# zhoubin-me/supertonic

Measured on AMD Instinct MI355X. Metric: audio-sec/sec (RTF^-1), 66M model, batch=128 per GPU, higher is better.
Workload: dtype bf16

## Files before the change

include/stn.h:

```cpp
#ifndef STN_H
#define STN_H
#include <stddef.h>
#include <stdint.h>

#include "stn_arch.h"

#ifdef __cplusplus
extern "C" {
#endif

#define STN_OK 0
#define STN_ERR_INVALID (-1)
#define STN_ERR_DEVICE (-2)
#define STN_ERR_STATE (-3)
#define STN_ERR_UNSUPPORTED (-4)
#define STN_ERR_IO (-5)

#define STN_DTYPE_F32 0
#define STN_DTYPE_BF16 1
#define STN_DTYPE_F16 2

typedef struct stn_handle stn_handle;

typedef struct stn_config {
// ... 233 lines not shown
int stn_expander_curve(const stn_expander* c, int n, const double* in_db, double* out_db);
const char* stn_expander_error(const stn_expander* c, int rate_hz);

int stn_profile_enable(stn_handle* h, int on);
int stn_profile_reset(stn_handle* h);
int stn_profile_filter(stn_handle* h, const char* family_or_null);
int stn_profile_sample(stn_handle* h, int every);
int stn_launch_log_enable(stn_handle* h, int on);
int64_t stn_launch_log(stn_handle* h, char* out, size_t cap);
int stn_profile_count(stn_handle* h);
int stn_profile_get(stn_handle* h, int idx, char* name, size_t name_cap, double* total_ms, int64_t* launches,
                    double* flops, double* bytes);

int stn_dbg_xattn_hs_enable(stn_handle* h, int on);
int64_t stn_dbg_xattn_hs_stamps(stn_handle* h, unsigned long long* out, size_t cap);
int stn_dbg_fold_run_frames(const int32_t* latent_lengths, int B, int n_cu);

int stn_op_gemm(stn_handle* h, int dtype, int M, int N, int K, const float* A , const float* W ,
                const float* bias_or_null, int act , float* out );
int stn_op_gemm_ex(stn_handle* h, int dtype, int M, int N, int K, const float* A , const float* W , int mode, int act,
                   int out_dtype, int ldo, const float* bias_or_null, const float* gamma_or_null, const int32_t* len_or_null, int L,
                   const int32_t* row_b_or_null, const float* rowvec_or_null, int nseq, int nt, int tr, float* out, int64_t out_elems,
                   char* form, size_t form_cap);
int stn_dbg_gemm_form(int dtype, int M, int N, int K, int mode, int out_dtype, int ldo, int masked, int tr, char* out, size_t cap);
int stn_dbg_ffn_form(int dtype, int stage, int C, int I, int64_t M, int64_t gate_rows, int packed, int k, int max_dil, int mask,
                     int64_t min_rows, int64_t split_min_rows, int nt_hints, char* out, size_t cap);
int stn_op_gemm_bench(stn_handle* h, int dtype, int M, int N, int K, int mode, int iters, double* avg_ms);
int stn_op_gemm_phases(stn_handle* h, int dtype, int M, int N, int K, int mode, double* out6);
int stn_op_dwconv_ln(stn_handle* h, int dtype, int B, int L, int C, int k, int dil, const float* x,
                     const float* w , const float* bias, const float* ln_g, const float* ln_b, float* y);
int stn_op_dwconv_ln_ragged(stn_handle* h, int dtype, int B, int L, int C, int k, int dil, const float* x,
                            const float* w , const float* bias, const float* ln_g, const float* ln_b,
                            const int32_t* seqlen , float* y);
int stn_op_dwconv_ln_ex(stn_handle* h, int dtype, int B, int L, int C, int k, int dil, const float* x, int64_t x_rows,
                        const float* w_or_null , const float* bias_or_null, const float* ln_g, const float* ln_b,
                        const int32_t* seqlen_or_null, int packed, int ln_only, float* y, int64_t y_rows, char* form, size_t form_cap);
int stn_op_dwconv_ln_tail(stn_handle* h, int dtype, int B, int L, int C, int k, int dil, const float* x, int64_t x_rows,
                          const float* w , const float* bias, const float* ln_g, const float* ln_b, const int32_t* seqlen,
                          const float* tail , int T, int rf, float* y, int64_t y_rows, char* form, size_t form_cap);
int stn_dbg_dwconv_ln_form(int dtype, int B, int L, int C, int k, int packed, char* out, size_t cap);
int stn_op_fold_ln(stn_handle* h, int dtype, int M, int C, int S, const float* part, const float* b2, const float* gamma,
                   const float* rowvec_or_null, const int32_t* row_b_or_null, int nseq, const float* ln_g, const float* ln_b, float* x,
                   float* y);
int stn_op_layout(stn_handle* h, int which, int dtype, const int32_t* p, int n_p, const float* a, int64_t a_n, const float* b, int64_t b_n,
                  const float* c, int64_t c_n, const int64_t* ids, int64_t ids_n, const int32_t* len, int packed, float* out, int64_t out_n,
                  float* out2, int64_t out2_n, int32_t* iout, int64_t iout_n);
int stn_op_attention(stn_handle* h, int dtype, int B, int Lq, int Lk, int H, int dh, const float* q, const float* k,
                     const float* v, const int32_t* qlen_or_null, const int32_t* klen_or_null, int rope_mode, float* o);
int stn_op_attention_ex(stn_handle* h, int dtype, int B, int Lq, int Lk, int H, int dh, const float* q, int64_t q_elems, int ldq,
                        int q_col, float* kv, int64_t kv_elems, int ldk, int k_col, int v_col, float* o, int64_t o_elems, int ldo,
                        const int32_t* qlen_or_null, const int32_t* klen_or_null, const int32_t* q_off_or_null,
                        const int32_t* k_off_or_null, int rope_mode, int k_rotated, int rot_groups, int rot_stride, int rot_col,
                        char* form, size_t form_cap);
int stn_op_xattn_hs(stn_handle* h, int dtype, int M, const float* xn, const float* Wq, const float* bq_or_null, const float* Wo,
                    const float* kv, int64_t kv_elems, int ldk, int k_col, int B, int L, int Lk, const int32_t* qlen,
                    const int32_t* klen_or_null, const int32_t* k_off_or_null, int rope_mode, int pairs_mode, int64_t part_stride,
                    float* part, int64_t part_elems, int32_t* pairs_out_or_null, char* form, size_t form_cap);
int stn_dbg_attn_form(int kind, int dtype, int B, int Lq, int Lk, int H, int dh, int ldq, int ldk, int misaligned, char* out, size_t cap);
int stn_op_ffn(stn_handle* h, int M, int C, int I, const float* xn , const float* W1, const float* b1, const float* W2,
               const float* b2_or_null, const float* gamma_or_null, const float* rowvec_or_null ,
               const int32_t* row_b_or_null , int nseq, float* x, int fused);
int stn_op_ffn_ex(stn_handle* h, int dtype, int M, int C, int I, const float* xn, int ldx, int64_t xn_elems, const float* W1, const float* b1,
                  const float* W2, const float* b2_or_null, const float* gamma_or_null, const int32_t* len_or_null, int L,
                  const int32_t* row_b_or_null, const float* rowvec_or_null, int rv_ld, int nseq, int mode, int split, float* x, int ldo,
                  int64_t x_elems, float* part_or_null, int64_t part_stride, int64_t part_elems, char* form, size_t form_cap);
int stn_op_ffn_bench(stn_handle* h, int M, int C, int I, int fused, int iters, double* out5);
int stn_op_fold_dwconv_ln(stn_handle* h, int B, int C, int k, int dil, int S, const int32_t* seqlen, const float* x, const float* part,
                          const float* b2_or_null, const float* gamma_or_null, const float* rowvec_or_null , const float* w ,
                          const float* bias, const float* ln_g, const float* ln_b, float* x_out, float* y);
int stn_op_fold_dwconv_ln_ex(stn_handle* h, int dtype, int B, int L, int C, int k, int dil, int S, int run_frames, const int32_t* seqlen,
                             const float* x_in, int64_t x_rows, const float* part, int64_t part_stride, int64_t part_elems,
                             const float* b2_or_null, const float* gamma_or_null, const float* rowvec_or_null, int rv_ld,
// ... 18 lines not shown
```

supertonic_amd/binding.py:

```python
import ctypes
import os

import numpy as np

from .arch import StnArch

_HERE = os.path.dirname(os.path.abspath(__file__))
LIB_PATH = os.environ.get("STN_LIB") or os.path.join(_HERE, "libstn.so")
_LIB = None

F32, BF16, F16 = 0, 1, 2
_DTYPES = {"f32": F32, "fp32": F32, "float32": F32, "bf16": BF16, "f16": F16, "fp16": F16, "float16": F16, "half": F16,
           F32: F32, BF16: BF16, F16: F16}
ACT_NONE, ACT_GELU, ACT_SILU, ACT_GELU_TANH = 0, 1, 2, 3
EPI_STORE, EPI_RESID, EPI_STORE_T = 0, 1, 2
FFN_VOCODER, FFN_ESTIMATOR, FFN_TEXT = 1, 2, 4
LAYOUT_ROW_MAP, LAYOUT_NCL_TO_ROWS, LAYOUT_EULER_NCL, LAYOUT_UNPACK_ROWS, LAYOUT_EMBED, LAYOUT_MASKED_MEAN, LAYOUT_IM2COL, LAYOUT_VOCODER_IN = range(8)
ENC_F32, ENC_PCM16, ENC_PCM24, ENC_MULAW, ENC_ALAW = 0, 1, 2, 3, 4
ENCODINGS = {"f32": ENC_F32, "pcm16": ENC_PCM16, "pcm24": ENC_PCM24, "mulaw": ENC_MULAW, "alaw": ENC_ALAW}
ENCODING_NAMES = {v: k for k, v in ENCODINGS.items()}
ENCODING_BYTES = {ENC_F32: 4, ENC_PCM16: 2, ENC_PCM24: 3, ENC_MULAW: 1, ENC_ALAW: 1}
ZERO_CODEWORD = {ENC_F32: 0, ENC_PCM16: 0, ENC_PCM24: 0, ENC_MULAW: 0xFF, ENC_ALAW: 0xD5}


def encoding_id(enc):
    if isinstance(enc, str) and enc.lower() in ENCODINGS:
        return ENCODINGS[enc.lower()]
    if not isinstance(enc, str) and int(enc) in ENCODING_NAMES:
        return int(enc)
    raise ValueError(f"unknown sample encoding {enc!r}: one of {', '.join(ENCODINGS)}")


def encoded_empty(enc, rows, W):
    e = encoding_id(enc)
    if e == ENC_PCM24:
        return np.empty((rows, W, 3), np.uint8)
    return np.empty((rows, W), {ENC_F32: np.float32, ENC_PCM16: np.int16}.get(e, np.uint8))


JOIN_WHOLE, JOIN_TRIM = 0, 1
JOIN_MODES = {"whole": JOIN_WHOLE, "trim": JOIN_TRIM, JOIN_WHOLE: JOIN_WHOLE, JOIN_TRIM: JOIN_TRIM}
JOIN_GAIN_ROW, JOIN_GAIN_PROG = 0, 1
JOIN_SCOPES = {"row": JOIN_GAIN_ROW, "programme": JOIN_GAIN_PROG, "prog": JOIN_GAIN_PROG, JOIN_GAIN_ROW: JOIN_GAIN_ROW, JOIN_GAIN_PROG: JOIN_GAIN_PROG}


class StnJoin(ctypes.Structure):
    _fields_ = [("n_prog", ctypes.c_int32), ("rows", ctypes.c_void_p), ("gap_samples", ctypes.c_void_p), ("gap_seconds", ctypes.c_void_p),
                ("mode", ctypes.c_int32), ("gain_scope", ctypes.c_int32)]


# ... 489 lines not shown
    L.stn_batch_copy_wav_device.argtypes = [vp, vp, ctypes.c_int64]
    L.stn_batch_copy_pcm16_device.argtypes = [vp, vp, ctypes.c_int64]
    L.stn_profile_filter.argtypes = [vp, ctypes.c_char_p]
    L.stn_profile_sample.argtypes = [vp, ci]
    L.stn_launch_log_enable.argtypes = [vp, ci]
    L.stn_dbg_xattn_hs_enable.argtypes = [vp, ci]
    L.stn_dbg_xattn_hs_stamps.argtypes = [vp, vp, ctypes.c_size_t]
    L.stn_dbg_xattn_hs_stamps.restype = ctypes.c_int64
    L.stn_dbg_fold_run_frames.argtypes = [vp, ctypes.c_int, ctypes.c_int]
    L.stn_dbg_fold_run_frames.restype = ctypes.c_int
    L.stn_dbg_gemm_form.argtypes = [ci, ci, ci, ci, ci, ci, ci, ci, ci, ctypes.c_char_p, ctypes.c_size_t]
    L.stn_dbg_gemm_form.restype = ctypes.c_int
    L.stn_dbg_attn_form.argtypes = [ci, ci, ci, ci, ci, ci, ci, ci, ci, ci, ctypes.c_char_p, ctypes.c_size_t]
    L.stn_dbg_attn_form.restype = ctypes.c_int
    L.stn_dbg_ffn_form.argtypes = [ci, ci, ci, ci, ctypes.c_int64, ctypes.c_int64, ci, ci, ci, ci, ctypes.c_int64, ctypes.c_int64, ci,
                                   ctypes.c_char_p, ctypes.c_size_t]
    L.stn_dbg_ffn_form.restype = ctypes.c_int
    L.stn_launch_log.argtypes = [vp, ctypes.c_char_p, ctypes.c_size_t]
    L.stn_launch_log.restype = ctypes.c_int64
    L.stn_profile_enable.argtypes = [vp, ci]
    L.stn_profile_reset.argtypes = [vp]
    L.stn_profile_count.argtypes = [vp]
    L.stn_profile_get.argtypes = [vp, ci, ctypes.c_char_p, ctypes.c_size_t, ctypes.POINTER(ctypes.c_double),
                                  ctypes.POINTER(ctypes.c_int64), ctypes.POINTER(ctypes.c_double),
                                  ctypes.POINTER(ctypes.c_double)]
    L.stn_op_gemm.argtypes = [vp, ci, ci, ci, ci, _f32p, _f32p, vp, ci, _f32p]
    L.stn_op_gemm_ex.argtypes = [vp, ci, ci, ci, ci, _f32p, _f32p, ci, ci, ci, ci, vp, vp, vp, ci, vp, vp, ci, ci, ci, _f32p,
                                 ctypes.c_int64, ctypes.c_char_p, ctypes.c_size_t]
    L.stn_op_gemm_bench.argtypes = [vp, ci, ci, ci, ci, ci, ci, ctypes.POINTER(ctypes.c_double)]
    L.stn_op_gemm_phases.argtypes = [vp, ci, ci, ci, ci, ci, ctypes.POINTER(ctypes.c_double)]
    L.stn_op_dwconv_ln.argtypes = [vp, ci, ci, ci, ci, ci, ci, _f32p, _f32p, _f32p, _f32p, _f32p, _f32p]
    L.stn_op_dwconv_ln_ragged.argtypes = [vp, ci, ci, ci, ci, ci, ci, _f32p, _f32p, _f32p, _f32p, _f32p, _i32p, _f32p]
    L.stn_op_attention.argtypes = [vp, ci, ci, ci, ci, ci, ci, _f32p, _f32p, _f32p, vp, vp, ci, _f32p]
    L.stn_op_dwconv_ln_ex.argtypes = [vp, ci, ci, ci, ci, ci, ci, _f32p, ctypes.c_int64, vp, vp, _f32p, _f32p, vp, ci, ci, _f32p, ctypes.c_int64,
                                      ctypes.c_char_p, ctypes.c_size_t]
    L.stn_op_dwconv_ln_tail.argtypes = [vp, ci, ci, ci, ci, ci, ci, _f32p, ctypes.c_int64, _f32p, _f32p, _f32p, _f32p, _i32p, _f32p, ci, ci, _f32p,
                                        ctypes.c_int64, ctypes.c_char_p, ctypes.c_size_t]
    L.stn_dbg_resample_form.argtypes = [ci, ci, ctypes.c_int64, ctypes.c_char_p, ctypes.c_size_t]
    L.stn_dbg_resample_form.restype = ctypes.c_int
    L.stn_dbg_dwconv_ln_form.argtypes = [ci, ci, ci, ci, ci, ci, ctypes.c_char_p, ctypes.c_size_t]
    L.stn_dbg_dwconv_ln_form.restype = ctypes.c_int
    L.stn_op_fold_ln.argtypes = [vp, ci, ci, ci, ci, _f32p, _f32p, _f32p, vp, vp, ci, _f32p, _f32p, _f32p, _f32p]
    L.stn_op_layout.argtypes = [vp, ci, ci, _i32p, ci, vp, ctypes.c_int64, vp, ctypes.c_int64, vp, ctypes.c_int64, vp, ctypes.c_int64, vp, ci,
                                vp, ctypes.c_int64, vp, ctypes.c_int64, vp, ctypes.c_int64]
    L.stn_op_attention_ex.argtypes = [vp, ci, ci, ci, ci, ci, ci, _f32p, ctypes.c_int64, ci, ci, _f32p, ctypes.c_int64, ci, ci, ci,
                                      _f32p, ctypes.c_int64, ci, vp, vp, vp, vp, ci, ci, ci, ci, ci, ctypes.c_char_p, ctypes.c_size_t]
    L.stn_op_xattn_hs.argtypes = [vp, ci, ci, _f32p, _f32p, vp, _f32p, _f32p, ctypes.c_int64, ci, ci, ci, ci, ci, _i32p, vp, vp, ci, ci,
                                  ctypes.c_int64, _f32p, ctypes.c_int64, vp, ctypes.c_char_p, ctypes.c_size_t]
    L.stn_op_randn.argtypes = [vp, cu64, ci, ci, ci, vp, vp, _f32p]
    L.stn_op_ffn.argtypes = [vp, ci, ci, ci, _f32p, _f32p, _f32p, _f32p, vp, vp, vp, vp, ci, _f32p, ci]
    L.stn_op_ffn_ex.argtypes = [vp, ci, ci, ci, ci, _f32p, ci, ctypes.c_int64, _f32p, _f32p, _f32p, vp, vp, vp, ci, vp, vp, ci, ci, ci, ci, _f32p, ci,
                                ctypes.c_int64, vp, ctypes.c_int64, ctypes.c_int64, ctypes.c_char_p, ctypes.c_size_t]
    L.stn_op_ffn_bench.argtypes = [vp, ci, ci, ci, ci, ci, ctypes.POINTER(ctypes.c_double)]
    L.stn_set_fused_ffn.argtypes = [vp, ci]
    L.stn_set_fused_ffn_min_rows.argtypes = [vp, ctypes.c_int64, ctypes.c_int64]
    L.stn_op_fold_dwconv_ln.argtypes = [vp, ci, ci, ci, ci, ci, _i32p, _f32p, _f32p, vp, vp, vp, _f32p, _f32p, _f32p, _f32p, _f32p, _f32p]
    L.stn_op_fold_dwconv_ln_ex.argtypes = [vp, ci, ci, ci, ci, ci, ci, ci, ci, _i32p, _f32p, ctypes.c_int64, _f32p, ctypes.c_int64, ctypes.c_int64, vp, vp,
                                           vp, ci, _f32p, _f32p, _f32p, _f32p, _f32p, ctypes.c_int64, _f32p, ctypes.c_int64, ctypes.c_char_p,
                                           ctypes.c_size_t]
    L.stn_dbg_fold_dwconv_ln_form.argtypes = [ci, ci, ci, ci, ci, ci, ci, ci, ci, ctypes.c_char_p, ctypes.c_size_t]
    L.stn_dbg_fold_dwconv_ln_form.restype = ctypes.c_int
    L.stn_op_block_bench.argtypes = [vp, ci, ci, ci, ci, ci, ci, ci, ci, ctypes.POINTER(ctypes.c_double)]
    L.stn_group_create.argtypes = [ci, vp, ci, ctypes.POINTER(vp)]
    L.stn_group_destroy.argtypes = [vp]
    L.stn_group_last_error.restype = ctypes.c_char_p
    L.stn_group_last_error.argtypes = [vp]
    L.stn_group_size.argtypes = [vp]
    L.stn_group_uses_rccl.argtypes = [vp]
    L.stn_group_handle.restype = vp
    L.stn_group_handle.argtypes = [vp, ci]
    L.stn_group_load_synthetic.argtypes = [vp, ctypes.POINTER(StnArch), cu64]
    L.stn_group_load_dir.argtypes = [vp, ctypes.c_char_p]
    L.stn_group_deal.argtypes = [ci, _i32p, ci, _i32p, _i32p]
    L.stn_group_synthesize.argtypes = [vp, ci, ci, _i64p, _f32p, _f32p, _f32p, ci, cf, vp, cu64, ctypes.POINTER(ctypes.c_int64)]
# ... 527 lines not shown
    r = load().stn_dbg_fold_run_frames(a.ctypes.data, len(a), int(n_cu))
    if r < 0:
        raise StnError(r, "stn_dbg_fold_run_frames: bad arguments")
    return int(r)


def gemm_form(dtype, M, N, K, mode=EPI_STORE, out_dtype="f32", ldo=None, masked=False, tr=-1):
    buf = ctypes.create_string_buffer(128)
    r = load().stn_dbg_gemm_form(_DTYPES[dtype], int(M), int(N), int(K), int(mode), _DTYPES[out_dtype], int(N if ldo is None else ldo),
                                 int(bool(masked)), int(tr), buf, len(buf))
    if r < 0:
        raise StnError(r, "stn_dbg_gemm_form: the launcher refuses this call")
    return buf.value.decode()


def attn_form(dtype, B, Lq, Lk, H, dh, ldq=None, ldk=None, misaligned=0, kind=0):
    buf = ctypes.create_string_buffer(64)
    C = H * dh
    r = load().stn_dbg_attn_form(int(kind), _DTYPES[dtype], int(B), int(Lq), int(Lk), int(H), int(dh), int(C if ldq is None else ldq),
                                 int(C if ldk is None else ldk), int(misaligned), buf, len(buf))
    if r < 0:
        raise StnError(r, "stn_dbg_attn_form: the launcher refuses this call")
    return buf.value.decode()


def dwconv_ln_form(dtype, B, L, C, k, packed=False):
    buf = ctypes.create_string_buffer(32)
    r = load().stn_dbg_dwconv_ln_form(_DTYPES[dtype], int(B), int(L), int(C), int(k), int(bool(packed)), buf, len(buf))
    if r < 0:
        raise StnError(r, "stn_dbg_dwconv_ln_form: the launcher refuses this call")
    return buf.value.decode()


def fold_dwconv_ln_form(dtype, B, L, C, k, dil, S, rowvec=True, run_frames=0):
    buf = ctypes.create_string_buffer(96)
    r = load().stn_dbg_fold_dwconv_ln_form(_DTYPES[dtype], int(B), int(L), int(C), int(k), int(dil), int(S), int(bool(rowvec)), int(run_frames),
                                           buf, len(buf))
    if r < 0:
        raise StnError(r, "stn_dbg_fold_dwconv_ln_form: the launcher refuses this call")
    return buf.value.decode()


def ffn_form(dtype, stage, C, I, M, gate_rows=0, packed=True, k=5, max_dil=1, mask=9, min_rows=18432, split_min_rows=1, nt_hints=True):
    buf = ctypes.create_string_buffer(32)
    r = load().stn_dbg_ffn_form(_DTYPES[dtype], int(stage), int(C), int(I), int(M), int(gate_rows), int(bool(packed)), int(k), int(max_dil),
                                int(mask), int(min_rows), int(split_min_rows), int(bool(nt_hints)), buf, len(buf))
    if r < 0:
        raise StnError(r, "stn_dbg_ffn_form: invalid arguments")
    return buf.value.decode()


def _c(a, dt):
    return np.ascontiguousarray(a, dtype=dt)


def _opt(a, dt):
    if a is None:
        return None, None
    arr = _c(a, dt)
    return arr, arr.ctypes.data


class Engine:

    def __init__(self, device=0, dtype="bf16"):
        self._lib = load()
# ... 903 lines not shown
        self._ck(self._lib.stn_op_fold_dwconv_ln_ex(self._h, self.dtype if dtype is None else _DTYPES[dtype], len(seqlen), int(L), C, w.shape[1], int(dil),
                                                    int(S), int(run_frames), seqlen, x_in.reshape(-1), x_in.shape[0], part, int(part_stride), part.size,
                                                    b2p, gp, vp_, C if _v is None else _v.shape[1], w, _c(bias, np.float32), _c(g, np.float32),
                                                    _c(b, np.float32), xo.reshape(-1), xo.shape[0], yo.reshape(-1), yo.shape[0], form, ctypes.sizeof(form)))
        return xo, yo, form.value.decode()

    def op_block_bench(self, B, L, C, I, k, dil, mode, iters=20):
        out = (ctypes.c_double * 6)()
        self._ck(self._lib.stn_op_block_bench(self._h, B, L, C, I, k, dil, mode, iters, out))
        return dict(ms=out[0], conv_ms=out[1], fold_phase1=out[2], fold_barrier=out[3], fold_phase2=out[4], fold_span=out[5])

    def set_fused_ffn_min_rows(self, k4_rows=-1, split_rows=-1):
        self._ck(self._lib.stn_set_fused_ffn_min_rows(self._h, int(k4_rows), int(split_rows)))

    def op_gemm_phases(self, M, N, K, mode=0, dtype=None):
        out = (ctypes.c_double * 6)()
        self._ck(self._lib.stn_op_gemm_phases(self._h, self.dtype if dtype is None else _DTYPES[dtype], M, N, K, mode, out))
        return dict(first_stage=out[0], k_loop=out[1], epilogue=out[2], grid_span=out[3], entry_spread=out[4], workgroups=int(out[5]))

    def op_dwconv_ln(self, x, w, bias, g, b, dil, dtype=None, seqlen=None):
        B, L, C = x.shape
        k = w.shape[1]
        y = np.empty((B, L, C), np.float32)
        if seqlen is not None:
            self._ck(self._lib.stn_op_dwconv_ln_ragged(self._h, self.dtype if dtype is None else _DTYPES[dtype], B, L, C, k,
                                                       dil, _c(x, np.float32), _c(w, np.float32), _c(bias, np.float32),
                                                       _c(g, np.float32), _c(b, np.float32), _c(seqlen, np.int32), y))
            return y
        self._ck(self._lib.stn_op_dwconv_ln(self._h, self.dtype if dtype is None else _DTYPES[dtype], B, L, C, k, dil,
                                            _c(x, np.float32), _c(w, np.float32), _c(bias, np.float32),
                                            _c(g, np.float32), _c(b, np.float32), y))
        return y

    def op_dwconv_ln_ex(self, x, w, bias, g, b, dil, out, B, L, seqlen=None, packed=False, ln_only=False, dtype=None):
        x = _c(x, np.float32)
        o_r = np.array(out, dtype=np.float32, order="C", copy=True)
        C = x.shape[1]
        _w, wp = _opt(w, np.float32)
        _b, bp = _opt(bias, np.float32)
        _l, lp = _opt(seqlen, np.int32)
        form = ctypes.create_string_buffer(32)
        self._ck(self._lib.stn_op_dwconv_ln_ex(self._h, self.dtype if dtype is None else _DTYPES[dtype], int(B), int(L), C,
                                               1 if _w is None else _w.shape[1], int(dil), x.reshape(-1), x.shape[0], wp, bp, _c(g, np.float32),
                                               _c(b, np.float32), lp, int(bool(packed)), int(bool(ln_only)), o_r.reshape(-1), o_r.shape[0], form,
                                               ctypes.sizeof(form)))
        return o_r, form.value.decode()

    def op_dwconv_ln_tail(self, x, w, bias, g, b, dil, out, L, seqlen, tail, T, dtype=None):
        x = _c(x, np.float32)
        tail = _c(tail, np.float32)
        o_r = np.array(out, dtype=np.float32, order="C", copy=True)
        C = x.shape[1]
        w = _c(w, np.float32)
        seqlen = _c(seqlen, np.int32)
        assert tail.ndim == 2 and tail.shape[1] == C and tail.shape[0] >= 1
        form = ctypes.create_string_buffer(32)
        self._ck(self._lib.stn_op_dwconv_ln_tail(self._h, self.dtype if dtype is None else _DTYPES[dtype], len(seqlen), int(L), C, w.shape[1],
                                                 int(dil), x.reshape(-1), x.shape[0], w, _c(bias, np.float32), _c(g, np.float32),
                                                 _c(b, np.float32), seqlen, tail.reshape(-1), int(T), tail.shape[0] - 1, o_r.reshape(-1),
                                                 o_r.shape[0], form, ctypes.sizeof(form)))
        return o_r, form.value.decode()

    def op_fold_ln(self, x, part, b2, gamma, g, b, rowvec=None, row_b=None, dtype=None):
        x_r = np.array(x, dtype=np.float32, order="C", copy=True)
        M, C = x_r.shape
        part = _c(part, np.float32)
# ... 91 lines not shown
```

supertonic_amd/csrc/api.cpp:

```cpp
#include "../../include/stn.h"

#include <algorithm>
#include <complex>
#include <cstdio>
#include <cstring>
#include <fstream>
#include <string>

#include "engine.hpp"
#include "host/json_min.hpp"
#include "host/graph_bind.hpp"
#include "host/onnx_reader.hpp"

#include <map>
#include <sstream>

struct stn_handle {
    stn::Engine* eng = nullptr;
    std::string err;
    std::vector<std::pair<std::string, stn::KernelStat>> prof;
};

static thread_local std::string g_create_err;

// ... 879 lines not shown
}
int stn_dbg_ffn_form(int dtype, int stage, int C, int I, int64_t M, int64_t gate_rows, int packed, int k, int max_dil, int mask,
                     int64_t min_rows, int64_t split_min_rows, int nt_hints, char* out, size_t cap) {
    if (C < 1 || I < 1 || M < 1 || k < 1 || max_dil < 1 || (stage != stn::FFN_VOCODER && stage != stn::FFN_ESTIMATOR && stage != stn::FFN_TEXT) ||
        (dtype != STN_DTYPE_F32 && dtype != STN_DTYPE_BF16 && dtype != STN_DTYPE_F16))
        return STN_ERR_INVALID;
    const std::string f = stn::ffn_form(dtype, stage, C, I, M, gate_rows, packed != 0, k, max_dil, mask, min_rows, split_min_rows, nt_hints != 0).str();
    if (out && cap > f.size()) std::memcpy(out, f.c_str(), f.size() + 1);
    return (int)f.size();
}
int stn_op_gemm_bench(stn_handle* h, int dtype, int M, int N, int K, int mode, int iters, double* avg_ms) {
    STN_TRY(h, { need(M > 0 && N > 0 && K > 0 && iters > 0 && avg_ms, "stn_op_gemm_bench: bad argument");
                 need(K % (dtype != STN_DTYPE_F32 ? 8 : 4) == 0, "K must be a multiple of 8 (bf16) / 4 (f32)");
                 *avg_ms = h->eng->op_gemm_bench(dtype, M, N, K, mode, iters); })
}
int stn_op_gemm_phases(stn_handle* h, int dtype, int M, int N, int K, int mode, double* out6) {
    STN_TRY(h, { need(M > 0 && N > 0 && K > 0 && out6, "stn_op_gemm_phases: bad argument");
                 need(K % (dtype != STN_DTYPE_F32 ? 8 : 4) == 0, "K must be a multiple of 8 (bf16) / 4 (f32)");
                 h->eng->op_gemm_phases(dtype, M, N, K, mode, out6); })
}
int stn_op_dwconv_ln(stn_handle* h, int dtype, int B, int L, int C, int k, int dil, const float* x, const float* w,
                     const float* bias, const float* g, const float* b, float* y) {
    STN_TRY(h, { need(B > 0 && L > 0 && C > 0 && C % 4 == 0 && C <= 1024 && k > 0 && (k & 1) && dil > 0 && x && w && bias && g && b && y,
                      "stn_op_dwconv_ln: bad argument");
                 h->eng->op_dwconv_ln(dtype, B, L, C, k, dil, x, w, bias, g, b, y); })
}
int stn_op_dwconv_ln_ragged(stn_handle* h, int dtype, int B, int L, int C, int k, int dil, const float* x, const float* w,
                            const float* bias, const float* g, const float* b, const int32_t* seqlen, float* y) {
    STN_TRY(h, { need(B > 0 && L > 0 && C > 0 && C % 4 == 0 && C <= 1024 && k > 0 && (k & 1) && dil > 0 && x && w && bias && g && b && y && seqlen,
                      "stn_op_dwconv_ln_ragged: bad argument");
                 for (int i = 0; i < B; ++i) need(seqlen[i] >= 0 && seqlen[i] <= L, "stn_op_dwconv_ln_ragged: seqlen out of [0, L]");
                 h->eng->op_dwconv_ln(dtype, B, L, C, k, dil, x, w, bias, g, b, y, seqlen); })
}
static void dwconv_ln_ex_checked(stn_handle* h, int dtype, int B, int L, int C, int k, int dil, const float* x, int64_t x_rows, const float* w,
                                 const float* bias, const float* g, const float* b, const int32_t* seqlen, int packed, int ln_only, float* y,
                                 int64_t y_rows, char* form, size_t form_cap) {
    need(B > 0 && L > 0 && C > 0 && C % 4 == 0 && C <= 1024 && k > 0 && (k & 1) && dil > 0 && x && g && b && y && x_rows > 0 && y_rows > 0,
         "stn_op_dwconv_ln_ex: bad argument");
    need(dtype == STN_DTYPE_F32 || dtype == STN_DTYPE_BF16 || dtype == STN_DTYPE_F16, "stn_op_dwconv_ln_ex: unknown dtype");
    need(ln_only || (w && bias), "stn_op_dwconv_ln_ex: the conv needs w and bias");
    need(!(packed && ln_only), "stn_op_dwconv_ln_ex: ln_only takes no packed layout");
    need(!packed || (seqlen && B <= 1024), "stn_op_dwconv_ln_ex: packed rows need seqlen and B <= 1024");
    int64_t rows = (int64_t)B * L;
    if (seqlen && !ln_only) {
        int64_t tot = 0;
        for (int i = 0; i < B; ++i) { need(seqlen[i] >= 0 && seqlen[i] <= L, "stn_op_dwconv_ln_ex: seqlen out of [0, L]"); tot += seqlen[i]; }
        if (packed) rows = tot;
    }
    need(x_rows >= rows && y_rows >= rows, "stn_op_dwconv_ln_ex: x / y hold fewer rows than the launch addresses");
    const std::string f = h->eng->op_dwconv_ln_ex(dtype, B, L, C, k, dil, x, x_rows, w, bias, g, b, ln_only ? nullptr : seqlen, packed, ln_only, y, y_rows);
    if (form && form_cap) std::snprintf(form, form_cap, "%s", f.c_str());
}
int stn_op_dwconv_ln_ex(stn_handle* h, int dtype, int B, int L, int C, int k, int dil, const float* x, int64_t x_rows, const float* w,
                        const float* bias, const float* g, const float* b, const int32_t* seqlen, int packed, int ln_only, float* y,
                        int64_t y_rows, char* form, size_t form_cap) {
    STN_TRY(h, dwconv_ln_ex_checked(h, dtype, B, L, C, k, dil, x, x_rows, w, bias, g, b, seqlen, packed, ln_only, y, y_rows, form, form_cap))
}
static void dwconv_ln_tail_checked(stn_handle* h, int dtype, int B, int L, int C, int k, int dil, const float* x, int64_t x_rows, const float* w,
                                   const float* bias, const float* g, const float* b, const int32_t* seqlen, const float* tail, int T, int rf,
                                   float* y, int64_t y_rows, char* form, size_t form_cap) {
    need(B > 0 && B <= 1024 && L > 0 && C > 0 && C % 4 == 0 && C <= 512 && (k == 5 || k == 7) && dil > 0 && x && w && bias && g && b && y && seqlen &&
             x_rows > 0 && y_rows > 0,
         "stn_op_dwconv_ln_tail: bad argument");
    need(dtype == STN_DTYPE_F32 || dtype == STN_DTYPE_BF16 || dtype == STN_DTYPE_F16, "stn_op_dwconv_ln_tail: unknown dtype");
    need(tail && rf >= 0 && T >= L, "stn_op_dwconv_ln_tail: needs a tail table of rf + 1 >= 1 rows and T >= L");
    int64_t rows = 0;
    for (int i = 0; i < B; ++i) { need(seqlen[i] >= 0 && seqlen[i] <= L, "stn_op_dwconv_ln_tail: seqlen out of [0, L]"); rows += seqlen[i]; }
    need(x_rows >= rows && y_rows >= rows, "stn_op_dwconv_ln_tail: x / y hold fewer rows than the launch addresses");
    const std::string f = h->eng->op_dwconv_ln_ex(dtype, B, L, C, k, dil, x, x_rows, w, bias, g, b, seqlen, 1, 0, y, y_rows, tail, T, rf);
    if (form && form_cap) std::snprintf(form, form_cap, "%s", f.c_str());
}
int stn_op_dwconv_ln_tail(stn_handle* h, int dtype, int B, int L, int C, int k, int dil, const float* x, int64_t x_rows, const float* w,
                          const float* bias, const float* g, const float* b, const int32_t* seqlen, const float* tail, int T, int rf, float* y,
                          int64_t y_rows, char* form, size_t form_cap) {
    STN_TRY(h, dwconv_ln_tail_checked(h, dtype, B, L, C, k, dil, x, x_rows, w, bias, g, b, seqlen, tail, T, rf, y, y_rows, form, form_cap))
}
int stn_dbg_dwconv_ln_form(int dtype, int B, int L, int C, int k, int packed, char* out, size_t cap) {
    if (B < 1 || L < 1 || C < 1 || k < 1 || !(k & 1) || (dtype != STN_DTYPE_F32 && dtype != STN_DTYPE_BF16 && dtype != STN_DTYPE_F16)) return STN_ERR_INVALID;
    std::string f;
    try { f = stn::dwconv_ln_form(dtype, B, L, C, k, packed != 0).str(); } catch (const std::exception&) { return STN_ERR_INVALID; }
    if (out && cap > f.size()) std::memcpy(out, f.c_str(), f.size() + 1);
    return (int)f.size();
}
int stn_op_fold_ln(stn_handle* h, int dtype, int M, int C, int S, const float* part, const float* b2, const float* gamma, const float* rowvec,
                   const int32_t* row_b, int nseq, const float* g, const float* b, float* x, float* y) {
    STN_TRY(h, { need(M > 0 && C > 0 && C % 4 == 0 && C <= 1024 && (S == 4 || S == 8 || S == 12 || S == 24) && part && b2 && gamma && g && b && x && y,
                      "stn_op_fold_ln: bad argument");
                 need(dtype == STN_DTYPE_BF16 || dtype == STN_DTYPE_F16, "stn_op_fold_ln: a 16-bit format needed");
                 need(!rowvec || nseq > 0, "stn_op_fold_ln: rowvec needs nseq > 0");
                 if (rowvec && row_b) for (int m = 0; m < M; ++m) need(row_b[m] >= 0 && row_b[m] < nseq, "stn_op_fold_ln: row_b out of range");
                 h->eng->op_fold_ln(dtype, M, C, S, part, b2, gamma, rowvec, row_b, nseq, g, b, x, y); })
}
int stn_op_layout(stn_handle* h, int which, int dtype, const int32_t* p, int n_p, const float* a, int64_t a_n, const float* b, int64_t b_n,
                  const float* c, int64_t c_n, const int64_t* ids, int64_t ids_n, const int32_t* len, int packed, float* out, int64_t out_n,
                  float* out2, int64_t out2_n, int32_t* iout, int64_t iout_n) {
    static const int n_params[8] = {3, 4, 5, 3, 4, 3, 6, 6};
    STN_TRY(h, { need(which >= 0 && which < 8 && p && n_p == n_params[which], "stn_op_layout: unknown kernel or parameter count");
                 need(dtype == STN_DTYPE_F32 || dtype == STN_DTYPE_BF16 || dtype == STN_DTYPE_F16, "stn_op_layout: unknown dtype");
                 need(a_n >= 0 && b_n >= 0 && c_n >= 0 && ids_n >= 0 && out_n >= 0 && out2_n >= 0 && iout_n >= 0 && (a || !a_n) && (b || !b_n) && (c || !c_n) &&
                          (ids || !ids_n) && (out || !out_n) && (out2 || !out2_n) && (iout || !iout_n),
                      "stn_op_layout: a buffer without a pointer");
                 h->eng->op_layout(which, dtype, p, a, a_n, b, b_n, c, c_n, ids, ids_n, len, packed, out, out_n, out2, out2_n, iout, iout_n); })
}
int stn_op_attention(stn_handle* h, int dtype, int B, int Lq, int Lk, int H, int dh, const float* q, const float* k,
                     const float* v, const int32_t* qlen, const int32_t* klen, int rope_mode, float* o) {
    STN_TRY(h, { need(B > 0 && Lq > 0 && Lk > 0 && H > 0 && dh >= 8 && dh % 8 == 0 && dh <= 96 && q && k && v && o,
                      "stn_op_attention: bad argument");
                 h->eng->op_attention(dtype, B, Lq, Lk, H, dh, q, k, v, qlen, klen, rope_mode, o); })
}
static void attention_ex_checked(stn_handle* h, int dtype, int B, int Lq, int Lk, int H, int dh, const float* q, int64_t q_elems, int ldq,
                                 int q_col, float* kv, int64_t kv_elems, int ldk, int k_col, int v_col, float* o, int64_t o_elems, int ldo,
                                 const int32_t* qlen, const int32_t* klen, const int32_t* q_off, const int32_t* k_off, int rope_mode,
                                 int k_rotated, int rot_groups, int rot_stride, int rot_col, char* form, size_t form_cap) {
    need(B > 0 && Lq > 0 && Lk > 0 && H > 0 && dh >= 8 && dh % 8 == 0 && dh <= 96 && q && kv && o, "stn_op_attention_ex: bad argument");
    need(dtype == STN_DTYPE_F32 || dtype == STN_DTYPE_BF16 || dtype == STN_DTYPE_F16, "stn_op_attention_ex: unknown dtype");
    need(rope_mode >= -1 && rope_mode <= 1, "stn_op_attention_ex: rope_mode must be -1, 0 or 1");
    const int64_t C = (int64_t)H * dh;
    need(ldq > 0 && ldk > 0 && ldo >= C && q_col >= 0 && k_col >= 0 && v_col >= 0 && q_col + C <= ldq && k_col + C <= ldk && v_col + C <= ldk,
         "stn_op_attention_ex: the heads must lie inside the rows (col + H*dh <= ld, ldo >= H*dh)");
    need((q_off == nullptr || qlen) && (k_off == nullptr || klen), "stn_op_attention_ex: packed rows need their lengths");
    const int64_t qrows = q_elems / ldq, krows = kv_elems / ldk, orows = o_elems / ldo;
    for (int b = 0; b < B; ++b) {
        need(!qlen || qlen[b] >= 0, "stn_op_attention_ex: qlen < 0");
        need(!klen || klen[b] >= 0, "stn_op_attention_ex: klen < 0");
        if (q_off)
            need(qlen[b] <= Lq && q_off[b] >= 0 && (int64_t)q_off[b] + qlen[b] <= std::min(qrows, orows),
                 "stn_op_attention_ex: packed query rows outside q / o (or qlen > Lq)");
        if (k_off) need(k_off[b] >= 0 && (int64_t)k_off[b] + std::min(klen[b], Lk) <= krows, "stn_op_attention_ex: packed key rows outside kv");
    }
    if (!q_off) need((int64_t)B * Lq <= std::min(qrows, orows), "stn_op_attention_ex: q / o hold fewer than B*Lq rows");
// ... 168 lines not shown
```

supertonic_amd/csrc/engine.cpp:

```cpp
#include "engine.hpp"
#include "dev_env.hpp"
#include "engine_internal.hpp"

#include <algorithm>
#include <cmath>
#include <cstdio>
#include <cstring>

namespace stn {
using detail::up;

Arena::~Arena() {
    for (auto& c : chunks_) (void)hipFree(c.p);
}
size_t Arena::capacity() const {
    size_t t = 0;
    for (auto& c : chunks_) t += c.cap;
    return t;
}
void* Arena::alloc(size_t bytes) {
    bytes = (bytes + 255) & ~size_t(255);
    if (bytes == 0) bytes = 256;
    for (;;) {
        if (cur_ < chunks_.size()) {
// ... 105 lines not shown
        if (g.exec2) (void)hipGraphExecDestroy(g.exec2);
        if (g.graph2) (void)hipGraphDestroy(g.graph2);
    }
    graphs_.clear();
    warm_keys_.clear();
}

void Engine::free_weights() {
    if (s_) (void)hipStreamSynchronize(s_);
    drop_graphs();
    ++wgen_;
    for (void* p : owned_) (void)hipFree(p);
    owned_.clear();
    w_.clear();
    frag_w_.clear();
    ffn_w_.clear();
    loaded_ = false;
    params_ = 0;
}

Engine::~Engine() {
    (void)hipSetDevice(device_);
    if (s_) (void)hipStreamSynchronize(s_);
    if (dp_s_) (void)hipStreamSynchronize(dp_s_);
    if (te_s_) (void)hipStreamSynchronize(te_s_);
    free_weights();
    for (void* p : batch_owned_) (void)hipFree(p);
    for (void* p : batch_retired_) (void)hipFree(p);
    free_vocoder_constants();
    if (tcond_.buf) (void)hipFree(tcond_.buf);
    for (auto& sp : spans_) { (void)hipEventDestroy(sp.a); (void)hipEventDestroy(sp.b); }
    for (auto ev : ev_pool_) (void)hipEventDestroy(ev);
    drop_graphs();
    if (pin_llen_) (void)hipHostFree(pin_llen_);
    if (pin_seed_) (void)hipHostFree(pin_seed_);
    if (seed_dev_) (void)hipFree(seed_dev_);
    rs_release();
    fl_release();
    xp_release();
    ds_release();
    cp_release();
    lo_release();
    for (auto& f : fetch_) {
        if (f.busy && f.done) (void)hipEventSynchronize(f.done);
        if (f.dev) (void)hipFree(f.dev);
        if (f.pin) (void)hipHostFree(f.pin);
        if (f.ready) (void)hipEventDestroy(f.ready);
        if (f.done) (void)hipEventDestroy(f.done);
    }
    if (copy_s_) (void)hipStreamDestroy(copy_s_);
    if (own_s_) (void)hipStreamDestroy(own_s_);
    if (dp_s_) (void)hipStreamDestroy(dp_s_);
    if (te_s_) (void)hipStreamDestroy(te_s_);
    if (ev_te_) (void)hipEventDestroy(ev_te_);
    if (ev_copied_) (void)hipEventDestroy(ev_copied_);
    if (ev_dp_) (void)hipEventDestroy(ev_dp_);
}

DevTensor& Engine::tensor(const std::string& name) {
    auto it = w_.find(name);
    if (it == w_.end()) throw std::runtime_error("unknown weight tensor: " + name);
    return it->second;
}
Linear Engine::linear(const std::string& p) {
    Linear l;
    l.w = tensor(p + ".w");
    l.b = tensor(p + ".b").f32;
    l.N = l.w.rows;
    l.K = l.w.cols;
// ... 548 lines not shown
float* Engine::ve_time_cond_dev(int rows, const float* total_step, const float* current_step, float* tb_out) {
    stage_ = "ve";
    const stn_arch& a = a_;
    const int C = a.ve_dim, nb = a.ve_main_blocks;
    float* tb = tb_out ? tb_out : f32_alloc((int64_t)rows * nb * C);
    const Arena::Mark mk = ar_.mark();
    float* te = f32_alloc((int64_t)rows * a.ve_time_dim);
    launch_time_embed(s_, current_step, total_step, rows, a.ve_time_dim, a.time_scale, te);
    float* t1 = f32_alloc((int64_t)rows * C);
    Epilogue et1; et1.mode = EPI_STORE; et1.act = ACT_SILU; et1.out_dtype = F32; et1.out = t1; et1.ldo = C;
    gemm("gemm_small_f32", F32, te, a.ve_time_dim, linear("ve.t1"), rows, et1);
    float* tc = f32_alloc((int64_t)rows * C);
    Epilogue et2; et2.mode = EPI_STORE; et2.out_dtype = F32; et2.out = tc; et2.ldo = C;
    gemm("gemm_small_f32", F32, t1, C, linear("ve.t2"), rows, et2);
    Epilogue et3; et3.mode = EPI_STORE; et3.out_dtype = F32; et3.out = tb; et3.ldo = nb * C;
    gemm("gemm_small_f32", F32, tc, C, linear("ve.time_all"), rows, et3);
    ar_.release(mk);
    return tb;
}

void Engine::ve_step_dev(int B, int L, const VeCtx& c, const float* noisy, const int* tlen, const int* llen,
                         const float* total_step, const float* current_step, float* denoised, const float* tb, const Ragged* rg,
                         const float* dt, void* z_rows, bool z_ready, bool z_next) {
    stage_ = "ve";
    const stn_arch& a = a_;
    const int C = a.ve_dim, D = a.latent_dim * a.chunk_compress_factor, nb = a.ve_main_blocks, H = a.ve_heads;
    const int64_t M = rg ? (int64_t)rg->rows : (int64_t)B * L;
    const int* rmask = rg ? nullptr : llen;
    const int* roff = rg ? rg->off : nullptr;
    const size_t esz = is_half(dt_) ? 2 : 4;
    const Arena::Mark mk = ar_.mark();
    const int Dp = (D + 63) / 64 * 64;
    void* z = z_rows ? z_rows : act_alloc(M * Dp);
    if (!(z_rows && z_ready)) launch_ncl_to_rows(s_, dt_, noisy, B, D, L, z, Dp, llen, roff);
    const FfnForm ff = ffn_plan(FFN_ESTIMATOR, C, a.ve_hidden, M, 0, rg != nullptr, a.ve_kernel, 1 << std::max(0, a.ve_dilated - 1));
    const bool split = ff.kind == FFN_K4_SPLIT;
    FoldState fs;
    fs.x = f32_alloc(M * C);
    if (split) {
        fs.x_alt = f32_alloc(M * C);
        fs.part_stride = ffn_split_rows(M) * C;
        fs.part = act_alloc(fs.part_stride * std::max(ff.split, H));
    }
    FoldState* const fsp = split ? &fs : nullptr;
    Epilogue ein; ein.mode = EPI_STORE; ein.out_dtype = F32; ein.out = fs.x; ein.ldo = C; ein.len = rmask; ein.L = L;
    gemm("gemm_in", dt_, z, Dp, linear("ve.in_pad"), (int)M, ein);
    if (!tb) tb = ve_time_cond_dev(B, total_step, current_step);

    auto cross = [&](const std::string& p, const void* kv_all, int blk, int Lk, const int* klen, int rope_mode) {
        const Attn w = attn_w(p, false);
        const char* kp0 = static_cast<const char*>(kv_all) + (size_t)blk * 2 * C * esz;
        const auto fq = frag_w_.find(w.q.w.as(dt_));
        const auto foa = frag_acc_w_.find(w.o.w.as(dt_));
        if (fused_xattn_ && split && unit_vec_ && C <= 1024 && fq != frag_w_.end() && foa != frag_acc_w_.end() && xattn_hs_supported(dt_, C, H, L, Lk, nb * 2 * C)) {
            const Arena::Mark m2 = ar_.mark();
            void* xn = act_alloc(M * C);
            fold_layernorm(fs, M, C, w.ln, xn, "layernorm");
            if (kv_all == c.text_kv && text_gate_) { auto fire = std::move(text_gate_); text_gate_ = nullptr; fire(); }
            if (prof_on_) prof_begin("xattn_hs", 4.0 * M * (double)C * C + 4.0 * M * (double)Lk * C,
                                     (double)M * C * (esz + 2.0 * H) + 2.0 * C * C * esz + (double)B * Lk * 2 * C * esz);
            unsigned long long* ts = nullptr;
            if (hs_ts_ && (int64_t)(B + 8) * H <= HS_TS_WG) { ts = hs_ts_; hs_ts_wgs_ = (B + 8) * H; }
            launch_xattn_hs(s_, dt_, xn, M, fq->second, w.q.b, kp0, kp0 + (size_t)C * esz, nb * 2 * C, foa->second, fs.part, fs.part_stride, B, L, Lk,
                            llen, klen, roff, kv_all == c.text_kv ? c.text_off : nullptr, rope_mode, a.rope_base, a.larope_gamma, ts, rg->hs_pairs);
            if (prof_on_) prof_end();
            fs.pending = true;
            fs.fold = FoldArgs{};
// ... 18 lines not shown
                         a.larope_gamma, rope_mode >= 0, roff, kv_all == c.text_kv ? c.text_off : nullptr);
        if (prof_on_) prof_end();
        Epilogue eo; eo.mode = EPI_RESID; eo.resid = x; eo.ldo = C; eo.len = rmask; eo.L = L;
        gemm("gemm_attn_out", dt_, o, C, w.o, (int)M, eo);
        ar_.release(m2);
    };

    for (int blk = 0; blk < nb; ++blk) {
        const std::string p = "ve.m" + std::to_string(blk);
        for (int j = 0; j < a.ve_dilated; ++j) {
            const bool last = j == a.ve_dilated - 1;
            convnext(convnext_w(p + ".dil" + std::to_string(j)), ff, fs.x, B, L, C, a.ve_hidden, a.ve_kernel, 1 << j, llen, nullptr,
                     last ? tb + (size_t)blk * C : nullptr, nb * C, rg, fsp);
        }
        if (a.ve_dilated == 0) launch_add_rowvec(s_, fs.x, tb + (size_t)blk * C, nb * C, B, L, C, llen);
        convnext(convnext_w(p + ".cn_a"), ff, fs.x, B, L, C, a.ve_hidden, a.ve_kernel, 1, llen, nullptr, nullptr, 0, rg, fsp);
        cross(p + ".text", c.text_kv, blk, c.Lt, tlen, 1);
        convnext(convnext_w(p + ".cn_b"), ff, fs.x, B, L, C, a.ve_hidden, a.ve_kernel, 1, llen, nullptr, nullptr, 0, rg, fsp);
        cross(p + ".style", c.style_kv, blk, a.n_style_ttl, nullptr, -1);
    }
    for (int j = 0; j < a.ve_tail_blocks; ++j)
        convnext(convnext_w("ve.tail" + std::to_string(j)), ff, fs.x, B, L, C, a.ve_hidden, a.ve_kernel, 1, llen, nullptr, nullptr, 0, rg, fsp);
    void* xn = act_alloc(M * C);
    fold_layernorm(fs, M, C, lnorm("ve.out_ln"), xn, nullptr);
    const float* dtv = dt;
    if (!dtv) {
        float* d = f32_alloc(B);
        launch_reciprocal(s_, total_step, B, d);
        dtv = d;
    }
    float* vel = f32_alloc(M * D);
    Epilogue eo; eo.mode = EPI_STORE; eo.out_dtype = F32; eo.out = vel; eo.ldo = D;
    gemm("gemm_out", dt_, xn, C, linear("ve.out"), (int)M, eo);
    launch_euler_ncl(s_, noisy, vel, dtv, llen, B, D, L, denoised, roff, (z_rows && z_next) ? z_rows : nullptr, dt_, Dp);
    ar_.release(mk);
}

int Engine::vocoder_receptive_field() const {
    int rf = (a_.vo_in_kernel - 1) / 2;
    for (int i = 0; i < a_.vo_blocks; ++i) rf += (a_.vo_kernel - 1) / 2 * a_.vo_dilations[i];
    return rf;
}

void Engine::hs_stamps_enable(bool on) {
    sync();
    drop_graphs();
    if (on && !hs_ts_) {
        void* d = nullptr;
        STN_HIP(hipMalloc(&d, sizeof(unsigned long long) * 8 * HS_TS_WG));
        STN_HIP(hipMemset(d, 0, sizeof(unsigned long long) * 8 * HS_TS_WG));
        hs_ts_ = static_cast<unsigned long long*>(d);
    } else if (!on && hs_ts_) {
        (void)hipFree(hs_ts_);
        hs_ts_ = nullptr;
    }
    hs_ts_wgs_ = 0;
}
int64_t Engine::hs_stamps_fetch(unsigned long long* out, size_t cap) {
    if (!hs_ts_) return 0;
    sync();
    const size_t n = std::min(cap, (size_t)hs_ts_wgs_ * 8);
    if (out && n) STN_HIP(hipMemcpy(out, hs_ts_, n * sizeof(unsigned long long), hipMemcpyDeviceToHost));
    return hs_ts_wgs_;
}

void Engine::prepare_xattn_weights() {
    frag_w_.clear();
// ... 117 lines not shown
}

int Engine::trimmed_rows(int B, int L, std::vector<int>* n_host) const {
    if (!packed_ve_ || vo_ragged_ || !vo_c_[0].quiet || vo_rf_ <= 0 || B > 1024) return 0;
    const int ccf = a_.chunk_compress_factor, T = L * ccf, rf = vo_rf_;
    long tot = 0;
    bool any = false;
    for (int i = 0; i < B; ++i) {
        const int l6 = bt_.h_llen[i] * ccf;
        const bool trim = l6 + 2 * rf <= T;
        any = any || trim;
        const int n = trim ? l6 + 2 * rf : T;
        if (n_host) n_host->push_back(n);
        tot += n;
    }
    return (any && tot * 10 <= (long)B * T * 9) ? (int)tot : 0;
}

int Engine::tail_rows(int B, int L) const {
    if (!packed_ve_ || vo_ragged_ || !vo_c_[0].tail || vo_rf_ <= 0 || B > 1024) return 0;
    const int ccf = a_.chunk_compress_factor, T = L * ccf, rf = vo_rf_;
    long tot = 0;
    for (int i = 0; i < B; ++i) tot += std::min(bt_.h_llen[i] * ccf + rf, T);
    return tot * 10 <= (long)B * T * 9 ? (int)tot : 0;
}

int Engine::vocoder_rows(int B, int L, int* form) const {
    int rows = trimmed_rows(B, L, nullptr);
    *form = rows ? VO_TRIM_2RF : VO_DENSE;
    if (!rows && (rows = tail_rows(B, L))) *form = VO_TRIM_TAIL;
    return rows;
}

void Engine::vocoder_dev(int B, int L, const float* latent, float* wav, const int* vlen, int vrows, const int* valid, bool tails) {
    stage_ = "vo";
    const stn_arch& a = a_;
    const int C = a.vo_dim, T = L * a.chunk_compress_factor;
    const bool packed = vlen && vrows > 0 && is_half(dt_) && B <= 1024 && dwconv_ln_supports_packed(C, a.vo_kernel);
    if (valid && !packed) throw std::runtime_error("trimmed vocoder needs the packed bf16 path");
    if (tails && !valid) throw std::logic_error("vocoder_dev: the tail form is a trimmed form");
    const int64_t M = packed ? (int64_t)vrows : (int64_t)B * T;
    const Arena::Mark mk = ar_.mark();
    Ragged rg;
    if (packed) {
        int* off = static_cast<int*>(ar_.alloc(sizeof(int) * (size_t)(B + 1)));
        launch_row_map(s_, vlen, B, off, nullptr);
        rg.off = off; rg.rows = vrows;
    }
    const Ragged* rgp = packed ? &rg : nullptr;
    float* x = f32_alloc(M * C);
    if (is_half(dt_)) {
        const int kp = (a.latent_dim * a.vo_in_kernel + 63) / 64 * 64;
        void* cols = act_alloc(M * kp);
        launch_vocoder_im2col(s_, dt_, latent, B, L, a.latent_dim, a.chunk_compress_factor, a.vo_in_kernel, kp, cols, vlen,
                              packed ? rg.off : nullptr);
        Linear lin;
        lin.w = tensor("vo.in_gemm.w"); lin.b = vecf("vo.in.b"); lin.N = C; lin.K = kp;
        Epilogue ei; ei.mode = EPI_STORE; ei.out_dtype = F32; ei.out = x; ei.ldo = C;
        gemm("gemm_in", dt_, cols, kp, lin, (int)M, ei);
    } else {
        if (prof_on_) prof_begin("vocoder_in", 2.0 * M * C * a.latent_dim * a.vo_in_kernel, (double)M * (a.latent_dim + C) * 4.0);
        launch_vocoder_in(s_, latent, B, L, a.latent_dim, a.chunk_compress_factor, vecf("vo.in.wt"), vecf("vo.in.b"), C,
                          a.vo_in_kernel, x, vlen);
        if (prof_on_) prof_end();
    }
    FfnForm ff = ffn_plan(FFN_VOCODER, C, a.vo_hidden, M, valid ? (int64_t)B * T : 0, packed, a.vo_kernel,
                          a.vo_blocks ? *std::max_element(a.vo_dilations, a.vo_dilations + a.vo_blocks) : 1);
    if (vo_force_ffn_ >= 0) ff = FfnForm{vo_force_ffn_, 1, false};
    const VoConsts& vc = vo_c_[ff.kind == FFN_K4];
    if (valid && !(vc.quiet && vc.edge && vc.tail)) throw std::logic_error("vocoder_dev: no zero-latent constants for form " + ff.str());
    DwconvTail tl;
    for (int i = 0; i < a.vo_blocks; ++i) {
        if (vo_capture_) {
            const int rf = vocoder_receptive_field();
            for (int j = 0; j <= rf; ++j)
                STN_HIP(hipMemcpyAsync(vo_capture_ + ((size_t)i * (rf + 1) + j) * C, x + (size_t)(M - 1 - j) * C, sizeof(float) * (size_t)C,
                                       hipMemcpyDeviceToDevice, s_));
        }
        if (tails) { tl.tail = vc.tail + (size_t)i * (vo_rf_ + 1) * C; tl.T = T; tl.rf = vo_rf_; }
        convnext(convnext_w("vo.blk" + std::to_string(i)), ff, x, B, T, C, a.vo_hidden, a.vo_kernel, a.vo_dilations[i],
                 packed ? vlen : nullptr, packed ? nullptr : vlen, nullptr, 0, rgp, nullptr, tl);
    }
    void* xn = act_alloc(M * C);
    const LNorm ln = lnorm("vo.out_ln");
    launch_layernorm(s_, dt_, x, M, C, ln.g, ln.b, a.ln_eps, xn);
    if (packed) {
        float* wp = f32_alloc(M * a.base_chunk_size);
        Epilogue e; e.mode = EPI_STORE; e.out_dtype = F32; e.out = wp; e.ldo = a.base_chunk_size;
        gemm("gemm_head", dt_, xn, C, linear("vo.head"), (int)M, e);
        if (prof_on_) prof_begin("unpack_rows", 0.0, ((double)M + (double)B * T) * a.base_chunk_size * 4.0);
        if (valid) launch_unpack_rows_quiet(s_, wp, valid, rg.off, B, T, a.base_chunk_size, vo_rf_, vc.quiet, vc.edge, wav);
        else launch_unpack_rows(s_, wp, vlen, rg.off, B, T, a.base_chunk_size, wav);
        if (prof_on_) prof_end();
    } else {
        Epilogue e; e.mode = EPI_STORE; e.out_dtype = F32; e.out = wav; e.ldo = a.base_chunk_size; e.len = vlen; e.L = T;
        gemm("gemm_head", dt_, xn, C, linear("vo.head"), (int)M, e);
    }
    ar_.release(mk);
}


void Engine::duration(int B, int Lt, const int64_t* ids, const float* style_dp, const float* text_mask, float* dur) {
    STN_HIP(hipSetDevice(device_));
    ar_.reset();
    int64_t* d_ids = up(ar_, s_, ids, (size_t)B * Lt);
    float* d_mask = up(ar_, s_, text_mask, (size_t)B * Lt);
    float* d_st = up(ar_, s_, style_dp, (size_t)B * a_.n_style_dp * a_.d_style_dp);
    int* tlen = static_cast<int*>(ar_.alloc(sizeof(int) * B));
    float* d_dur = f32_alloc(B);
    launch_mask_to_len(s_, d_mask, B, Lt, tlen);
    duration_dev(B, Lt, d_ids, d_st, tlen, d_dur);
    STN_HIP(hipMemcpyAsync(dur, d_dur, sizeof(float) * B, hipMemcpyDeviceToHost, s_));
    sync();
}

void Engine::text_enc(int B, int Lt, const int64_t* ids, const float* style_ttl, const float* text_mask, float* text_emb) {
    STN_HIP(hipSetDevice(device_));
    ar_.reset();
    int64_t* d_ids = up(ar_, s_, ids, (size_t)B * Lt);
    float* d_mask = up(ar_, s_, text_mask, (size_t)B * Lt);
    float* d_st = up(ar_, s_, style_ttl, (size_t)B * a_.n_style_ttl * a_.d_style_ttl);
    int* tlen = static_cast<int*>(ar_.alloc(sizeof(int) * B));
    const size_t n = (size_t)B * a_.te_out_dim * Lt;
    float* d_out = f32_alloc(n);
    launch_mask_to_len(s_, d_mask, B, Lt, tlen);
    text_enc_dev(B, Lt, d_ids, d_st, tlen, d_out, nullptr);
// ... 44 lines not shown
```

supertonic_amd/csrc/engine.hpp:

```cpp
#pragma once
#include <cmath>
#include <hip/hip_runtime.h>

#include <cstdint>
#include <functional>
#include <iterator>
#include <stdexcept>
#include <string>
#include <unordered_map>
#include <vector>

#include "../../include/stn_arch.h"
#include "host/join_plan.hpp"
#include "host/pause_plan.hpp"
#include "host/pitch.hpp"
#include "kernels.hpp"

namespace stn {

#define STN_HIP(expr)                                                                                          \
    do {                                                                                                       \
        hipError_t e_ = (expr);                                                                                \
        if (e_ != hipSuccess)                                                                                  \
            throw std::runtime_error(std::string("HIP error: ") + hipGetErrorString(e_) + " at " #expr);       \
    } while (0)

struct DevTensor {
    float* f32 = nullptr;
    uint16_t* bf16 = nullptr;
    int rows = 0, cols = 0;
    const void* as(int dt) const { return is_half(dt) ? static_cast<const void*>(bf16) : static_cast<const void*>(f32); }
};

struct Linear { DevTensor w; const float* b = nullptr; int N = 0, K = 0; };
struct LNorm { const float* g = nullptr; const float* b = nullptr; };
struct ConvNeXt { const float* dw_t = nullptr; const float* dw_b = nullptr; LNorm ln; Linear pw1, pw2; const float* gamma = nullptr; };
struct Attn { LNorm ln; Linear q, kv, qkv, o; };

class Arena {
   public:
    struct Mark { size_t chunk, off; };
    Arena() = default;
    Arena(const Arena&) = delete;
    Arena& operator=(const Arena&) = delete;
    ~Arena();
// ... 76 lines not shown
    void load_synthetic(const stn_arch& a, uint64_t seed);
    using TensorSource = std::function<std::vector<float>(const std::string& name, int rows, int cols)>;
    void load_tensors(const stn_arch& a, const TensorSource& src);
    std::vector<std::string> tensor_names(const stn_arch& a);
    bool loaded() const { return loaded_; }
    const stn_arch& arch() const { return a_; }
    int64_t param_count() const { return params_; }
    int dtype() const { return dt_; }
    hipStream_t stream() const { return s_; }
    void sync() { STN_HIP(hipStreamSynchronize(s_)); if (dp_s_) STN_HIP(hipStreamSynchronize(dp_s_)); if (te_s_) STN_HIP(hipStreamSynchronize(te_s_)); }
    void set_stream(hipStream_t s);

    struct Ragged;
    void duration_dev(int B, int Lt, const int64_t* ids, const float* style_dp, const int* tlen, float* dur, const Ragged* trg = nullptr);
    void text_enc_dev(int B, int Lt, const int64_t* ids, const float* style_ttl, const int* tlen, float* ncl, void* rows,
                      const Ragged* trg = nullptr);
    struct VeCtx { void* text_kv = nullptr; void* style_kv = nullptr; int Lt = 0; const int* text_off = nullptr; };
    VeCtx ve_prepare_dev(int B, int Lt, const void* text_rows, const float* style_ttl, const int* tlen, const Ragged* trg = nullptr, bool defer_text = false);
    void ve_text_kv_dev(const VeCtx& c, int B, int Lt, const void* text_rows, const int* tlen, const Ragged* trg);
    float* ve_time_cond_dev(int rows, const float* total_step, const float* current_step, float* tb_out = nullptr );
    struct TimeCond { int steps = 0, B = 0; uint64_t wgen = ~0ull; float* buf = nullptr; size_t cap = 0; float *tot = nullptr, *cur = nullptr, *dt = nullptr, *tb = nullptr; };
    TimeCond tcond_;
    void ensure_time_cond(int total_step, int B);
    struct Ragged { const int* off = nullptr; const int* row_b = nullptr; int rows = 0;
                    const int* hs_pairs = nullptr;
                    int fold_run = 0; };
    void ve_step_dev(int B, int L, const VeCtx& c, const float* noisy, const int* tlen, const int* llen,
                     const float* total_step, const float* current_step, float* denoised, const float* tb = nullptr,
                     const Ragged* rg = nullptr, const float* dt = nullptr ,
                     void* z_rows = nullptr ,
                     bool z_ready = false ,
                     bool z_next = false );
    void vocoder_dev(int B, int L, const float* latent, float* wav, const int* vlen = nullptr, int vrows = 0,
                     const int* valid = nullptr, bool tails = false);
    int vocoder_receptive_field() const;
    void prepare_xattn_weights();
    std::unordered_map<const void*, const void*> frag_w_;
    void hs_stamps_enable(bool on);
    int64_t hs_stamps_fetch(unsigned long long* out, size_t cap);
    unsigned long long* hs_ts_ = nullptr;
    int hs_ts_wgs_ = 0;
    static constexpr int HS_TS_WG = 8192;
    const float* unit_vec_ = nullptr;
    std::unordered_map<const void*, const void*> frag_acc_w_;
    void prepare_vocoder_constants();
    void prepare_ffn_weights();
    struct FfnW { const void *wseq = nullptr, *wsplit[std::size(FFN_SPLITS)] = {}; };
    std::unordered_map<const void*, FfnW> ffn_w_;

    void duration(int B, int Lt, const int64_t* ids, const float* style_dp, const float* text_mask, float* dur);
    void text_enc(int B, int Lt, const int64_t* ids, const float* style_ttl, const float* text_mask, float* text_emb);
    void vector_est(int B, int L, int Lt, const float* noisy, const float* text_emb, const float* style_ttl,
                    const float* text_mask, const float* latent_mask, const float* total_step,
                    const float* current_step, float* denoised);
    void vocoder(int B, int L, const float* latent, float* wav);

    struct Batch {
        int B = 0, Lt = 0, L = 0, noise_L = 0, total_step = 0;
        float speed = 1.f;
        bool have_override = false, have_noise = false;
        uint64_t noise_seed = 0;
        int64_t* ids = nullptr; size_t ids_cap = 0;
        int* tlen = nullptr; size_t tlen_cap = 0;
        float* style_ttl = nullptr; size_t ttl_cap = 0;
        float* style_dp = nullptr; size_t dp_cap = 0;
        float* dur = nullptr; size_t dur_cap = 0;
        int* llen = nullptr; size_t llen_cap = 0;
        int64_t* utt_ids = nullptr; size_t utt_cap = 0;
        float* noise = nullptr; size_t noise_cap = 0;
        float* xt[2] = {nullptr, nullptr}; size_t xt_cap[2] = {0, 0};
        float* wav = nullptr; size_t wav_cap = 0;
        unsigned char* text_side = nullptr; size_t text_side_cap = 0;
        unsigned char* text_rows = nullptr; size_t text_cap = 0;
        int* toff = nullptr; size_t toff_cap = 0;
        int trows = 0;
        uint64_t gen = 0;
        std::vector<float> h_dur; std::vector<int> h_llen;
    };
    void batch_upload(int B, int Lt, const int64_t* ids, const float* text_mask, const float* style_ttl,
                      const float* style_dp, const float* duration_override, const int64_t* utt_ids);
    void batch_set_noise(const float* noise, int L);
    void batch_run(int total_step, float speed, uint64_t noise_seed);
    void set_graph_mode(bool on) { graph_on_ = on; }
    void set_vocoder_mode(bool length_aware) { vo_ragged_ = length_aware; }
    void set_packed_rows(bool on) { packed_ve_ = on; }
    void set_gelu_form(int tanh_form) { if ((tanh_form != 0) != (gelu_act_ == ACT_GELU_TANH)) { sync(); drop_graphs(); } gelu_act_ = tanh_form ? ACT_GELU_TANH : ACT_GELU; }
    int gelu_form() const { return gelu_act_ == ACT_GELU_TANH ? 1 : 0; }
    void set_shape_buckets(bool on) { shape_buckets_ = on; }
    static int64_t bucket_up(int64_t x, int64_t min_gran) {
        if (x <= 0) return x;
        int64_t g = min_gran;
        while (g * 8 <= x) g *= 2;
        return (x + g - 1) / g * g;
    }
    void set_duration_read(bool always) { dur_read_always_ = always; }
    void set_fused_xattn(int mode) { fused_xattn_ = mode ? 1 : 0; }
    void set_fused_ffn(int mask) { fused_ffn_ = mask; }
    void set_fused_ffn_min_rows(int64_t k4_rows, int64_t split_rows) {
        sync(); drop_graphs();
        if (k4_rows >= 0) ffn_min_rows_ = k4_rows;
// ... 146 lines not shown
    void set_expander(bool on, const stn_expander* c);
    bool expander_on() const { return xp_on_; }
    const stn_expander& expander() const { return xp_set_; }
    void batch_expander(float* min_attenuation_db, int64_t* closed_samples);
    struct XpProbe {
        int x_misalign = 0, in_place = 0;
        float *open = nullptr, *s1_end = nullptr, *s1_start = nullptr, *s2_end = nullptr, *s2_start = nullptr;
        bool guard_ok = false;
        const char* form = "";
    };
    void op_expander(int hz, int rows, int W, const float* x, const stn_expander& c, float* y, XpProbe* probe);

    void profile_enable(bool on) { if (on != prof_on_) profile_reset(); prof_on_ = on; }
    void launch_log_enable(bool on);
    std::string launch_log() const;
    void profile_sample(int every) { prof_every_ = every < 1 ? 1 : every; prof_seen_ = 0; }
    void profile_filter(const std::string& family) { if (family != prof_filter_) profile_reset(); prof_filter_ = family; }
    void profile_reset();
    std::vector<std::pair<std::string, KernelStat>> profile_collect();

    void op_gemm(int dtype, int M, int N, int K, const float* A, const float* W, const float* bias, int act, float* out);
    std::string op_gemm_ex(int dtype, int M, int N, int K, const float* A, const float* W, int mode, int act, int out_dtype, int ldo,
                           const float* bias, const float* gamma, const int* len, int L, const int* row_b, const float* rowvec, int nseq,
                           int nt, int tr, float* out, int64_t out_elems);
    std::string op_attention_ex(int dtype, int B, int Lq, int Lk, int H, int dh, const float* q, int64_t q_elems, int ldq, int q_col,
                                float* kv, int64_t kv_elems, int ldk, int k_col, int v_col, float* o, int64_t o_elems, int ldo,
                                const int* qlen, const int* klen, const int* q_off, const int* k_off, int rope_mode, int k_rotated,
                                int rot_groups, int rot_stride, int rot_col);
    std::string op_xattn_hs(int dtype, int M, const float* xn, const float* Wq, const float* bq, const float* Wo, const float* kv,
                            int64_t kv_elems, int ldk, int k_col, int B, int L, int Lk, const int* qlen, const int* klen, const int* k_off,
                            int rope_mode, int pairs_mode, int64_t part_stride, float* part, int64_t part_elems, int* pairs_out);
    void op_attention(int dtype, int B, int Lq, int Lk, int H, int dh, const float* q, const float* k, const float* v,
                      const int* qlen, const int* klen, int rope_mode, float* o);
    void op_dwconv_ln(int dtype, int B, int L, int C, int k, int dil, const float* x, const float* w, const float* bias,
                      const float* g, const float* b, float* y, const int* seqlen = nullptr );
    std::string op_dwconv_ln_ex(int dtype, int B, int L, int C, int k, int dil, const float* x, int64_t x_rows, const float* w, const float* bias,
                                const float* g, const float* b, const int* seqlen, int packed, int ln_only, float* y, int64_t y_rows,
                                const float* tail = nullptr, int T = 0, int rf = 0);
    void op_fold_ln(int dtype, int M, int C, int S, const float* part, const float* b2, const float* gamma, const float* rowvec, const int* row_b,
                    int nseq, const float* g, const float* b, float* x, float* y);
    void op_layout(int which, int dtype, const int* p, const float* a, int64_t a_n, const float* b, int64_t b_n, const float* c, int64_t c_n,
                   const int64_t* ids, int64_t ids_n, const int* len, int packed, float* out, int64_t out_n, float* out2, int64_t out2_n, int* iout,
                   int64_t iout_n);
    double op_gemm_bench(int dtype, int M, int N, int K, int mode, int iters);
    void op_gemm_phases(int dtype, int M, int N, int K, int mode, double* out6);
    void op_randn(uint64_t seed, int B, int D, int L, const int64_t* utt_ids, const int* len, float* out);
    void op_ffn(int M, int C, int I, const float* xn, const float* W1, const float* b1, const float* W2, const float* b2, const float* gamma,
                const float* rowvec , const int* row_b , int nseq, float* x, int mode);
    std::string op_ffn_ex(int M, int C, int I, const float* xn, int ldx, int64_t xn_elems, const float* W1, const float* b1, const float* W2,
                          const float* b2, const float* gamma, const int* len, int L, const int* row_b, const float* rowvec, int rv_ld, int nseq,
                          int mode, int split, float* x, int ldo, int64_t x_elems, float* part, int64_t part_stride, int64_t part_elems);
    void op_fold_dwconv_ln(int B, int C, int k, int dil, int S, const int* seqlen, const float* x, const float* part, const float* b2,
                           const float* gamma, const float* rowvec , const float* w , const float* bias,
                           const float* g, const float* b, float* x_out, float* y);
    std::string op_fold_dwconv_ln_ex(int dtype, int B, int L, int C, int k, int dil, int S, int run_frames, const int* seqlen, const float* x_in,
                                     int64_t x_rows, const float* part, int64_t part_stride, int64_t part_elems, const float* b2, const float* gamma,
                                     const float* rowvec, int rv_ld, const float* w, const float* bias, const float* g, const float* b, float* x_out,
                                     int64_t x_out_rows, float* y, int64_t y_rows);
    void op_ffn_bench(int M, int C, int I, int mode, int iters, double* out5);
    void op_block_bench(int B, int L, int C, int I, int k, int dil, int mode, int iters, double* out6);

    Arena& arena() { return ar_; }

   private:
    DevTensor& tensor(const std::string& name);
    const float* vecf(const std::string& name) { return tensor(name).f32; }
// ... 94 lines not shown
    void drop_graphs();
    bool graph_on_ = true;
    bool vo_ragged_ = false;
    bool packed_ve_ = true;
    bool nt_hints_ = true;
    hipStream_t dp_s_ = nullptr, te_s_ = nullptr;
    Arena dp_ar_, te_ar_;
    hipEvent_t ev_te_ = nullptr, ev_copied_ = nullptr, ev_dp_ = nullptr;
    std::function<void()> text_gate_;
    bool copied_valid_ = false;
    int64_t ffn_min_rows_ = 18432;
    int64_t ffn_split_min_rows_ = 1;
    int fused_ffn_ = 9;
    bool shape_buckets_ = false;
    bool dur_read_always_ = false;
    int gelu_act_ = ACT_GELU;
    int fused_xattn_ = 1;
    int64_t last_ve_rows_ = 0, last_vo_rows_ = 0;
    struct VoConsts {
        float* quiet = nullptr;
        float* edge = nullptr;
        float* tail = nullptr;
    };
    VoConsts vo_c_[2];
    int vo_rf_ = 0;
    int vo_force_ffn_ = -1;
    float* vo_capture_ = nullptr;
    void free_vocoder_constants();
    enum VoForm : int { VO_DENSE = 0, VO_TRIM_2RF = 1, VO_TRIM_TAIL = 2 };
    int trimmed_rows(int B, int L, std::vector<int>* n_host) const;
    int tail_rows(int B, int L) const;
    int vocoder_rows(int B, int L, int* form) const;
    long graph_replays_ = 0;
    int* pin_llen_ = nullptr; size_t pin_llen_cap_ = 0;
    unsigned long long* pin_seed_ = nullptr;
    bool pin_valid_ = false;
    unsigned long long* seed_dev_ = nullptr;
    int final_xt_ = 0;
    struct FetchSlot { unsigned char* dev = nullptr; unsigned char* pin = nullptr; size_t cap = 0, n = 0; int enc = ENC_PCM16; hipEvent_t ready = nullptr, done = nullptr; bool busy = false; std::vector<float> dur; };
    FetchSlot fetch_[2];
    int out_hz_ = 0;
    ResampleTable rs_, op_rs_;
    void rs_prepare(ResampleTable& t, int in_hz, int out_hz);
    const ResampleTable& rs_table();
    void rs_release();
    void resample_enqueue(const ResampleTable& t, const float* x, int64_t rows, int64_t W, int enc, void* y, int64_t dst_stride);
    float ps_semi_ = 0.0f;
    int ps_a_ = 1, ps_b_ = 1;
    uint64_t ps_gen_ = 0;
    ResampleTable ps_rs_, op_ps_rs_;
    void ps_table(ResampleTable& t, int a, int b);
    DevBuf ps_buf_;
    struct PsScratch { int64_t* n; float* win; int* delta; float* score; float* ys; float* y; size_t bytes; };
    static PsScratch ps_layout(char* base, int64_t rows, int64_t W, const PitchPlan& p);
    std::vector<int64_t> ps_n_; std::vector<float> ps_win_;
    struct PsKey {
        uint64_t seq = 0, gen = 0; int64_t W = 0; int B = 0; const void* buf = nullptr;
        bool operator==(const PsKey& o) const { return seq == o.seq && gen == o.gen && W == o.W && B == o.B && buf == o.buf; }
    };
    PsKey ps_key_; bool ps_valid_ = false;
    void ps_enqueue(const float* x, int64_t rows, int64_t W, const int64_t* n, int a, int b, const PitchPlan& p, const float* win, int* delta, float* score,
                    float* ys);
    void ps_resample(const ResampleTable& t, const float* ys, int64_t rows, int64_t Ws, int64_t W, float* y);
    void ps_op(int hz, int rows, int W, const float* x, const int64_t* n, int a, int b, float* ys_out, int* delta_out, float* score_out, float* y_out);
    const float* ps_batch();
    const float* wav_rows() { return pitch_on() ? ps_batch() : bt_.wav; }
    bool lo_on_ = false;
    float lo_target_ = -23.0f, lo_ceiling_ = -1.0f;
    LoudTable lo_, op_lo_;
// ... 177 lines not shown
```

supertonic_amd/csrc/engine_batch.cpp:

```cpp
#include "engine.hpp"
#include "engine_internal.hpp"

#include <algorithm>
#include <cmath>
#include <cstdio>
#include <cstring>

namespace stn {
using detail::up;


template <typename T>
void Engine::ensure(T*& p, size_t& cap, size_t need) {
    if (p && need <= cap) return;
    const size_t n = std::max<size_t>(need + need / 4, 64);
    T* q = nullptr;
    STN_HIP(hipMalloc(reinterpret_cast<void**>(&q), n * sizeof(T)));
    if (p) {
        batch_owned_.erase(std::find(batch_owned_.begin(), batch_owned_.end(), static_cast<void*>(p)));
        batch_retired_.push_back(p);
    }
    batch_owned_.push_back(q);
    p = q;
    cap = n;
    ++bt_.gen;
}

void Engine::batch_upload(int B, int Lt, const int64_t* ids, const float* text_mask, const float* style_ttl,
                          const float* style_dp, const float* duration_override, const int64_t* utt_ids) {
    STN_HIP(hipSetDevice(device_));
    if (!loaded_) throw std::runtime_error("no model loaded");
    if (B <= 0 || Lt <= 0) throw std::runtime_error("empty batch");
    sync();
    for (void* p : batch_retired_) (void)hipFree(p);
    batch_retired_.clear();
    Batch& b = bt_;
    const int Lt_in = Lt;
    if (shape_buckets_) Lt = (int)bucket_up(Lt, 32);
    b.B = B; b.Lt = Lt; b.L = 0; b.noise_L = 0; b.total_step = 0;
    b.have_override = false; b.have_noise = false;
    b.h_dur.clear(); b.h_llen.clear();
    const size_t n_ttl = (size_t)B * a_.n_style_ttl * a_.d_style_ttl, n_dp = (size_t)B * a_.n_style_dp * a_.d_style_dp;
    ensure(b.ids, b.ids_cap, (size_t)B * Lt);
    ensure(b.tlen, b.tlen_cap, (size_t)B);
    ensure(b.style_ttl, b.ttl_cap, n_ttl);
    ensure(b.style_dp, b.dp_cap, n_dp);
    ensure(b.dur, b.dur_cap, (size_t)B);
    ensure(b.llen, b.llen_cap, (size_t)B);
    ensure(b.utt_ids, b.utt_cap, (size_t)B);
    if (Lt != Lt_in) {
        STN_HIP(hipMemsetAsync(b.ids, 0, sizeof(int64_t) * B * Lt, s_));
        STN_HIP(hipMemcpy2DAsync(b.ids, sizeof(int64_t) * Lt, ids, sizeof(int64_t) * Lt_in, sizeof(int64_t) * Lt_in, (size_t)B, hipMemcpyHostToDevice, s_));
    } else {
        STN_HIP(hipMemcpyAsync(b.ids, ids, sizeof(int64_t) * B * Lt, hipMemcpyHostToDevice, s_));
    }
    STN_HIP(hipMemcpyAsync(b.style_ttl, style_ttl, sizeof(float) * n_ttl, hipMemcpyHostToDevice, s_));
    STN_HIP(hipMemcpyAsync(b.style_dp, style_dp, sizeof(float) * n_dp, hipMemcpyHostToDevice, s_));
    std::vector<int64_t> uid(B);
    for (int i = 0; i < B; ++i) uid[i] = utt_ids ? utt_ids[i] : i;
    STN_HIP(hipMemcpyAsync(b.utt_ids, uid.data(), sizeof(int64_t) * B, hipMemcpyHostToDevice, s_));
    ar_.reset();
    float* d_mask = up(ar_, s_, text_mask, (size_t)B * Lt_in);
    launch_mask_to_len(s_, d_mask, B, Lt_in, b.tlen);
    ensure(b.toff, b.toff_cap, (size_t)B + 1);
    b.trows = 0;
    for (int i = 0; i < B; ++i) {
        int n = 0;
        for (int t = 0; t < Lt_in; ++t) n += text_mask[(size_t)i * Lt_in + t] > 0.5f ? 1 : 0;
        b.trows += n;
    }
    if (shape_buckets_) b.trows = (int)bucket_up(b.trows, 64);
    if (B <= 1024) launch_row_map(s_, b.tlen, B, b.toff, nullptr);
    b.have_override = duration_override != nullptr;
    if (duration_override) b.h_dur.assign(duration_override, duration_override + B);
    sync();
}

void Engine::batch_set_noise(const float* noise, int L) {
    STN_HIP(hipSetDevice(device_));
    Batch& b = bt_;
    if (b.B == 0) throw std::runtime_error("batch_set_noise: no batch uploaded");
// ... 50 lines not shown
            STN_HIP(hipEventRecord(ev_te_, s_));
        }
        {
            Side side(*this, dp_s_, dp_ar_);
            duration_dev(B, Lt, b.ids, b.style_dp, b.tlen, b.dur, tpk ? &trg : nullptr);
            if (!b.have_override || dur_read_always_) {
                STN_HIP(hipMemcpyAsync(dur.data(), b.dur, sizeof(float) * B, hipMemcpyDeviceToHost, s_));
                STN_HIP(hipEventRecord(ev_dp_, s_));
            }
        }
        if (!b.have_override || dur_read_always_) STN_HIP(hipEventSynchronize(ev_dp_));
        if (b.have_override) dur = b.h_dur;
    }
    auto take_text_rows = [this, &b, text_bytes]() {
        if (te_s_) STN_HIP(hipStreamWaitEvent(s_, ev_te_, 0));
        STN_HIP(hipMemcpyAsync(b.text_rows, b.text_side, text_bytes, hipMemcpyDeviceToDevice, s_));
        STN_HIP(hipEventRecord(ev_copied_, s_));
        copied_valid_ = true;
    };
    for (float& d : dur) d /= speed;
    int L = 0;
    latent_geometry(a, dur, L, b.h_llen);
    if (L < 1) throw std::runtime_error("predicted duration too short: zero latent frames");
    if (shape_buckets_ && !b.have_noise) L = (int)bucket_up(L, 16);
    if (b.have_noise && b.noise_L != L)
        throw std::runtime_error("injected noise has L=" + std::to_string(b.noise_L) + " but the durations imply L=" + std::to_string(L));
    b.L = L;
    reported_dur_ = dur;
    ++ed_seq_;
    const size_t nx = (size_t)B * D * L, nw = (size_t)B * L * a.base_chunk_size * a.chunk_compress_factor;
    ensure(b.xt[0], b.xt_cap[0], nx);
    ensure(b.xt[1], b.xt_cap[1], nx);
    ensure(b.wav, b.wav_cap, nw);
    if ((size_t)B > pin_llen_cap_) {
        if (pin_llen_) { sync(); drop_graphs(); (void)hipHostFree(pin_llen_); pin_llen_ = nullptr; }
        const size_t cap = std::max<size_t>((size_t)B, 1024);
        STN_HIP(hipHostMalloc(reinterpret_cast<void**>(&pin_llen_), sizeof(int) * cap, hipHostMallocDefault));
        pin_llen_cap_ = cap;
        pin_valid_ = false;
    }
    if (!pin_seed_) {
        STN_HIP(hipHostMalloc(reinterpret_cast<void**>(&pin_seed_), sizeof(unsigned long long), hipHostMallocDefault));
        STN_HIP(hipMalloc(reinterpret_cast<void**>(&seed_dev_), sizeof(unsigned long long)));
        pin_valid_ = false;
    }
    if (!pin_valid_ || !std::equal(b.h_llen.begin(), b.h_llen.end(), pin_llen_) || *pin_seed_ != (unsigned long long)noise_seed) {
        sync();
        std::copy(b.h_llen.begin(), b.h_llen.end(), pin_llen_);
        *pin_seed_ = (unsigned long long)noise_seed;
        pin_valid_ = true;
    }

    ensure_time_cond(total_step, B);
    GraphKey key;
    key.B = B; key.Lt = Lt; key.L = L; key.steps = total_step; key.noise = b.have_noise; key.ragged = vo_ragged_; key.xattn = fused_xattn_;
    key.ffn = fused_ffn_; key.gen = b.gen; key.wgen = wgen_; key.pin = pin_llen_;
    key.rows = 0;
    if (packed_rows_ok(B)) for (int v : b.h_llen) key.rows += v;
    if (shape_buckets_) key.rows = (int)bucket_up(key.rows, 64);
    last_ve_rows_ = key.rows ? key.rows : (int64_t)B * L;
    key.vrows = vocoder_rows(B, L, &key.vform);
    if (shape_buckets_) key.vrows = (int)bucket_up(key.vrows, 64 * a.chunk_compress_factor);
    key.trows = tpk ? b.trows : 0;
    last_vo_rows_ = (int64_t)B * L * a.chunk_compress_factor;
    if (vo_ragged_ && packed_ve_ && is_half(dt_)) {
        last_vo_rows_ = 0;
        for (int v : b.h_llen) last_vo_rows_ += (int64_t)v * a.chunk_compress_factor;
        if (shape_buckets_) last_vo_rows_ = bucket_up(last_vo_rows_, 64 * a.chunk_compress_factor);
        key.vrows = (int)last_vo_rows_;
    }
    else if (key.vrows) last_vo_rows_ = key.vrows;
    key.p0 = b.xt[0]; key.p1 = b.wav; key.s = s_;
    const bool graphable = graph_on_ && !prof_on_;
    if (graphable) {
        for (auto& g : graphs_)
            if (g.key == key) {
                g.last_use = ++graph_clock_;
                STN_HIP(hipGraphLaunch(g.exec, s_));
                take_text_rows();
                STN_HIP(hipGraphLaunch(g.exec2, s_));
                ++graph_replays_;
                return;
            }
    }
    const auto warm = std::find(warm_keys_.begin(), warm_keys_.end(), key);
    if (graphable && warm != warm_keys_.end()) {
        const Arena::Mark cap0 = ar_.mark();
        const size_t cap_before = ar_.capacity();
        STN_HIP(hipStreamBeginCapture(s_, hipStreamCaptureModeThreadLocal));
        bool ok = true;
        std::string why;
        hipGraph_t g = nullptr, g2 = nullptr;
        hipError_t ec1 = hipErrorUnknown;
        bool split = false;
// ... 40 lines not shown
        warm_keys_.push_back(key);
    }
    enqueue_after_duration(total_step, take_text_rows);
}

void Engine::ensure_time_cond(int total_step, int B) {
    TimeCond& t = tcond_;
    if (t.steps == total_step && t.B == B && t.wgen == wgen_ && t.buf) return;
    const stn_arch& a = a_;
    const size_t n_cnt = (size_t)2 * total_step * B + (size_t)B, n_tb = (size_t)total_step * B * a.ve_main_blocks * a.ve_dim;
    const size_t need = (n_cnt + 3) / 4 * 4 + n_tb;
    if (need > t.cap) {
        sync();
        drop_graphs();
        if (t.buf) (void)hipFree(t.buf);
        t.buf = nullptr; t.cap = 0;
        STN_HIP(hipMalloc(reinterpret_cast<void**>(&t.buf), need * sizeof(float)));
        t.cap = need;
    }
    t.tot = t.buf; t.cur = t.tot + (size_t)total_step * B; t.dt = t.cur + (size_t)total_step * B; t.tb = t.buf + (n_cnt + 3) / 4 * 4;
    t.steps = 0;
    const Arena::Mark mk = ar_.mark();
    launch_step_counters(s_, t.tot, t.cur, t.dt, B, total_step);
    (void)ve_time_cond_dev(total_step * B, t.tot, t.cur, t.tb);
    ar_.release(mk);
    t.steps = total_step; t.B = B; t.wgen = wgen_;
}

void Engine::enqueue_after_duration(int total_step, const std::function<void()>& take_text_rows) {
    Batch& b = bt_;
    const stn_arch& a = a_;
    const int B = b.B, Lt = b.Lt, L = b.L, D = a.latent_dim * a.chunk_compress_factor;
    const size_t nx = (size_t)B * D * L;
    STN_HIP(hipMemcpyAsync(b.llen, pin_llen_, sizeof(int) * B, hipMemcpyHostToDevice, s_));
    STN_HIP(hipMemcpyAsync(seed_dev_, pin_seed_, sizeof(unsigned long long), hipMemcpyHostToDevice, s_));
    Ragged trg;
    const bool tpk = packed_text_ok(B) && b.trows > 0;
    if (tpk) { trg.off = b.toff; trg.rows = b.trows; }
    const Ragged* trgp = tpk ? &trg : nullptr;
    void* text_rows = b.text_rows;
    if (b.have_noise) {
        STN_HIP(hipMemcpyAsync(b.xt[0], b.noise, nx * 4, hipMemcpyDeviceToDevice, s_));
        launch_mask_ncl(s_, b.xt[0], B, D, L, b.llen);
    } else {
        launch_randn_masked(s_, 0, b.utt_ids, B, D, L, b.llen, b.xt[0], seed_dev_);
    }
    VeCtx c = ve_prepare_dev(B, Lt, text_rows, b.style_ttl, b.tlen, trgp, true);
    text_gate_ = [this, &c, &b, &take_text_rows, B, Lt, text_rows, trgp]() {
        take_text_rows();
        ve_text_kv_dev(c, B, Lt, text_rows, b.tlen, trgp);
    };
    struct Disarm { std::function<void()>& g; ~Disarm() { g = nullptr; } } disarm{text_gate_};
    if (a.ve_main_blocks == 0) { auto fire = std::move(text_gate_); text_gate_ = nullptr; fire(); }
    if (tcond_.steps != total_step || tcond_.B != B || tcond_.wgen != wgen_) throw std::runtime_error("time conditioning not prepared for this run");
    const float* tot_all = tcond_.tot;
    const float* cur_all = tcond_.cur;
    const float* dt_all = tcond_.dt;
    const float* tb_all = tcond_.tb;
    const size_t tb_stride = (size_t)B * a.ve_main_blocks * a.ve_dim;
    Ragged rg;
    const Ragged* rgp = nullptr;
    if (packed_rows_ok(B)) {
        rg.rows = 0;
        for (int v : b.h_llen) rg.rows += v;
        if (shape_buckets_) rg.rows = (int)bucket_up(rg.rows, 64);
        int* off = static_cast<int*>(ar_.alloc(sizeof(int) * (size_t)(B + 1)));
        int* row_b = static_cast<int*>(ar_.alloc(sizeof(int) * (size_t)std::max(rg.rows, 1)));
        launch_row_map(s_, b.llen, B, off, row_b, rg.rows);
        rg.off = off; rg.row_b = row_b;
        rg.fold_run = fold_run_frames(b.h_llen.data(), B, n_cu_);
        if (fused_xattn_ && is_half(dt_) && B >= 2) {
            int* pairs = static_cast<int*>(ar_.alloc(sizeof(int) * (size_t)(B + 2)));
            launch_xattn_hs_pairs(s_, b.llen, B, pairs);
            rg.hs_pairs = pairs;
        }
        rgp = &rg;
    }
    int cur = 0;
    const int Dz = (a.latent_dim * a.chunk_compress_factor + 63) / 64 * 64;
    const int64_t Mz = rgp ? (int64_t)rg.rows : (int64_t)B * L;
    void* z_rows = act_alloc(Mz * Dz);
    for (int st = 0; st < total_step; ++st) {
        ve_step_dev(B, L, c, b.xt[cur], b.tlen, b.llen, tot_all + (size_t)st * B, cur_all + (size_t)st * B, b.xt[cur ^ 1],
                    tb_all + (size_t)st * tb_stride, rgp, dt_all, z_rows, st > 0, st + 1 < total_step);
        cur ^= 1;
    }
    final_xt_ = cur;
    const int* vlen = nullptr;
    if (vo_ragged_) {
        int* v = static_cast<int*>(ar_.alloc(sizeof(int) * B));
        launch_scale_len(s_, b.llen, B, a.chunk_compress_factor, v);
        vlen = v;
    }
    int vrows = 0;
    const int* valid = nullptr;
    bool tails = false;
    if (vo_ragged_ && packed_ve_) {
        for (int v : b.h_llen) vrows += v * a.chunk_compress_factor;
        if (shape_buckets_) vrows = (int)bucket_up(vrows, 64 * a.chunk_compress_factor);
    } else if (int vform = VO_DENSE; int tr = vocoder_rows(B, L, &vform)) {
        if (shape_buckets_) tr = (int)bucket_up(tr, 64 * a.chunk_compress_factor);
        int* n_dev = static_cast<int*>(ar_.alloc(sizeof(int) * B));
        int* v_dev = static_cast<int*>(ar_.alloc(sizeof(int) * B));
        launch_trim_len(s_, b.llen, B, a.chunk_compress_factor, L * a.chunk_compress_factor, vo_rf_, n_dev, v_dev, vform == VO_TRIM_TAIL);
        vlen = n_dev; valid = v_dev; vrows = tr; tails = vform == VO_TRIM_TAIL;
    }
    vocoder_dev(B, L, b.xt[cur], b.wav, vlen, vrows, valid, tails);
    STN_HIP(hipGetLastError());
}


char* DevBuf::reserve(Engine& e, size_t bytes, bool* moved) {
    const bool grow = !p_ || bytes > cap_;
    if (moved) *moved = grow;
    if (!grow) return p_;
    e.sync();
    if (p_) (void)hipFree(p_);
    p_ = nullptr; cap_ = 0;
    STN_HIP(hipMalloc(reinterpret_cast<void**>(&p_), bytes + bytes / 4));
    cap_ = bytes + bytes / 4;
    return p_;
}

int64_t Engine::out_row_len() {
    STN_HIP(hipSetDevice(device_));
    const Batch& b = bt_;
    if (!b.wav || b.L == 0) throw std::runtime_error("no finished batch");
    return out_len(native_row_len());
}

bool Engine::out_native() const { return !pitch_on() && !loudness_on() && !out_in_scratch(); }

const float* Engine::out_source(int64_t Wo) {
    const Batch& b = bt_;
    const float* wav = wav_rows();
    if (!out_in_scratch()) return wav;
    float* d = out_f32_buf((size_t)b.B * Wo);
    if (resample_on()) resample_enqueue(rs_table(), wav, b.B, native_row_len(), ENC_F32, d, Wo);
    if (filter_on()) fl_batch(resample_on() ? d : wav, Wo, d);
    if (expander_on()) xp_batch(resample_on() || filter_on() ? d : wav, Wo, d);
// ... 442 lines not shown
```

supertonic_amd/csrc/engine_ops.cpp:

```cpp
#include "engine.hpp"
#include "engine_internal.hpp"

#include <algorithm>
#include <cmath>
#include <cstdio>
#include <cstring>

namespace stn {
using detail::up;

void Engine::op_gemm(int dtype, int M, int N, int K, const float* A, const float* W, const float* bias, int act, float* out) {
    STN_HIP(hipSetDevice(device_));
    ar_.reset();
    float* dA = up(ar_, s_, A, (size_t)M * K);
    float* dW = up(ar_, s_, W, (size_t)N * K);
    float* dB = bias ? up(ar_, s_, bias, (size_t)N) : nullptr;
    float* dO = f32_alloc((size_t)M * N);
    const void* pa = dA;
    const void* pw = dW;
    if (is_half(dtype)) {
        void* a16 = ar_.alloc((size_t)M * K * 2);
        void* w16 = ar_.alloc((size_t)N * K * 2);
        launch_cast(s_, dtype, dA, (int64_t)M * K, a16);
        launch_cast(s_, dtype, dW, (int64_t)N * K, w16);
// ... 14 lines not shown
    float* dA = up(ar_, s_, A, (size_t)M * K);
    float* dW = up(ar_, s_, W, (size_t)N * K);
    const void* pa = dA;
    const void* pw = dW;
    if (is_half(dtype)) {
        void* a16 = ar_.alloc((size_t)M * K * 2);
        void* w16 = ar_.alloc((size_t)N * K * 2);
        launch_cast(s_, dtype, dA, (int64_t)M * K, a16);
        launch_cast(s_, dtype, dW, (int64_t)N * K, w16);
        pa = a16; pw = w16;
    }
    float* dO = up(ar_, s_, out, (size_t)out_elems);
    void* o16 = nullptr;
    if (mode == EPI_STORE && out_dtype != F32) {
        o16 = ar_.alloc((size_t)out_elems * 2);
        launch_cast(s_, out_dtype, dO, out_elems, o16);
    }
    Epilogue e;
    e.mode = mode; e.act = act; e.out_dtype = mode == EPI_STORE ? out_dtype : F32; e.ldo = ldo;
    e.out = mode == EPI_RESID ? nullptr : (o16 ? o16 : static_cast<void*>(dO));
    e.resid = mode == EPI_RESID ? dO : nullptr;
    e.bias = bias ? up(ar_, s_, bias, (size_t)N) : nullptr;
    e.gamma = gamma ? up(ar_, s_, gamma, (size_t)N) : nullptr;
    e.len = len ? up(ar_, s_, len, (size_t)nseq) : nullptr;
    e.L = L;
    e.row_b = row_b ? up(ar_, s_, row_b, (size_t)M) : nullptr;
    e.rowvec = rowvec ? up(ar_, s_, rowvec, (size_t)nseq * N) : nullptr;
    e.rv_ld = N;
    e.nt = nt;
    e.tr_force = tr;
    const GemmForm f = gemm_form(dtype, M, N, K, K, K, e, pa, pw);
    launch_gemm_form(s_, f, pa, K, pw, K, M, N, K, e, f.split > 1 ? f32_alloc((int64_t)f.split * M * N) : nullptr);
    if (o16) launch_half_to_f32(s_, out_dtype, o16, out_elems, dO);
    STN_HIP(hipMemcpyAsync(out, dO, (size_t)out_elems * 4, hipMemcpyDeviceToHost, s_));
    sync();
    return f.str();
}

void Engine::op_dwconv_ln(int dtype, int B, int L, int C, int k, int dil, const float* x, const float* w, const float* bias,
                          const float* g, const float* b, float* y, const int* seqlen) {
    STN_HIP(hipSetDevice(device_));
    ar_.reset();
    const size_t n = (size_t)B * L * C;
    const int* dlen = seqlen ? up(ar_, s_, seqlen, (size_t)B) : nullptr;
    std::vector<float> wt((size_t)C * k);
    for (int c = 0; c < C; ++c) for (int j = 0; j < k; ++j) wt[(size_t)j * C + c] = w[(size_t)c * k + j];
    float* dx = up(ar_, s_, x, n);
    float* dw = up(ar_, s_, wt.data(), wt.size());
    float* db = up(ar_, s_, bias, (size_t)C);
    float* dg = up(ar_, s_, g, (size_t)C);
    float* dbt = up(ar_, s_, b, (size_t)C);
    void* dy = ar_.alloc(n * 4);
    float* dy32 = f32_alloc(n);
    launch_dwconv_ln(s_, dtype, dx, B, L, C, dw, db, k, dil, dg, dbt, 1e-6f, dy, dlen);
    if (is_half(dtype)) launch_half_to_f32(s_, dtype, dy, (int64_t)n, dy32);
    STN_HIP(hipMemcpyAsync(y, is_half(dtype) ? dy32 : static_cast<float*>(dy), n * 4, hipMemcpyDeviceToHost, s_));
    sync();
}

void Engine::op_attention(int dtype, int B, int Lq, int Lk, int H, int dh, const float* q, const float* k, const float* v,
                          const int* qlen, const int* klen, int rope_mode, float* o) {
    STN_HIP(hipSetDevice(device_));
    ar_.reset();
    const int C = H * dh;
    const size_t nq = (size_t)B * Lq * C, nk = (size_t)B * Lk * C;
    float* dq = up(ar_, s_, q, nq);
// ... 610 lines not shown
        void* da = up_as(ar_, s_, dtype, a, (size_t)a_n);
        float* d = up(ar_, s_, out, (size_t)out_n);
        launch_masked_mean(s_, dtype, da, B, L, C, dlen, d, row_off(dlen, B));
        STN_HIP(hipMemcpyAsync(out, d, (size_t)out_n * 4, hipMemcpyDeviceToHost, s_));
        break;
    }
    case 6: {
        const int B = p[0], L = p[1], ld = p[2], ccf = p[3], k = p[4], kp = p[5];
        need(L > 0 && ld > 0 && ccf > 0 && k > 0 && (k & 1) && kp > 0 && a && out, "vocoder_im2col: bad shape");
        check_len(B, L * ccf, false);
        need(a_n >= (int64_t)B * ld * ccf * L && out_n >= rows_needed(B, L * ccf) * kp, "vocoder_im2col: buffer too small");
        const int* dlen = len ? up(ar_, s_, len, (size_t)B) : nullptr;
        float* da = up(ar_, s_, a, (size_t)a_n);
        void* d = up_as(ar_, s_, dtype, out, (size_t)out_n);
        launch_vocoder_im2col(s_, dtype, da, B, L, ld, ccf, k, kp, d, dlen, row_off(dlen, B));
        down_as(ar_, s_, dtype, d, out, (size_t)out_n);
        break;
    }
    case 7: {
        const int B = p[0], L = p[1], ld = p[2], ccf = p[3], C = p[4], k = p[5];
        need(L > 0 && ld > 0 && ccf > 0 && C > 0 && k > 0 && (k & 1) && (int64_t)(8 + k - 1) * ld * 4 <= 64 * 1024 && a && b && c && out, "vocoder_in: bad shape");
        need(!packed, "vocoder_in: padded rows only");
        check_len(B, L * ccf, false);
        need(a_n >= (int64_t)B * ld * ccf * L && b_n >= (int64_t)ld * k * C && c_n >= C && out_n >= (int64_t)B * L * ccf * C, "vocoder_in: buffer too small");
        const int* dlen = len ? up(ar_, s_, len, (size_t)B) : nullptr;
        float* da = up(ar_, s_, a, (size_t)a_n);
        float* dw = up(ar_, s_, b, (size_t)b_n);
        float* db = up(ar_, s_, c, (size_t)c_n);
        float* d = up(ar_, s_, out, (size_t)out_n);
        launch_vocoder_in(s_, da, B, L, ld, ccf, dw, db, C, k, d, dlen);
        STN_HIP(hipMemcpyAsync(out, d, (size_t)out_n * 4, hipMemcpyDeviceToHost, s_));
        break;
    }
    default: need(false, "unknown kernel");
    }
    STN_HIP(hipGetLastError());
    sync();
}

void Engine::op_randn(uint64_t seed, int B, int D, int L, const int64_t* utt_ids, const int* len, float* out) {
    STN_HIP(hipSetDevice(device_));
    ar_.reset();
    int64_t* du = utt_ids ? up(ar_, s_, utt_ids, (size_t)B) : nullptr;
    int* dl = len ? up(ar_, s_, len, (size_t)B) : nullptr;
    float* d = f32_alloc((size_t)B * D * L);
    launch_randn_masked(s_, seed, du, B, D, L, dl, d);
    STN_HIP(hipMemcpyAsync(out, d, (size_t)B * D * L * 4, hipMemcpyDeviceToHost, s_));
    sync();
}

}
```

supertonic_amd/csrc/kernels.hpp:

```cpp
#pragma once
#include <hip/hip_runtime.h>
#include <hip/hip_ext.h>
#include <stdint.h>
#include <stdio.h>
#include <stdlib.h>

#include <stdexcept>
#include <type_traits>
#include <utility>
#include <vector>
#include <string>

#include "dither.hpp"

namespace stn {

struct LaunchEvents { hipEvent_t start = nullptr, stop = nullptr; };
inline thread_local LaunchEvents g_launch_ev;
struct LaunchLog {
    bool on = false;
    const char* family = "-";
    std::vector<std::pair<std::string, const char*>> entries;
    void add(const char* kexpr) { if (entries.size() < 200000) entries.emplace_back(family, kexpr); }
};
// ... 26 lines not shown
template <typename Fn>
inline void with_out_type(int dtype, Fn&& fn) {
    if (dtype == F16) fn(static_cast<f16_t*>(nullptr));
    else if (dtype == BF16) fn(static_cast<uint16_t*>(nullptr));
    else fn(static_cast<float*>(nullptr));
}
template <typename Fn>
inline void with_half_type(int dtype, Fn&& fn) {
    if (dtype == F16) fn(static_cast<f16_t*>(nullptr));
    else fn(static_cast<uint16_t*>(nullptr));
}
enum ActFn : int { ACT_NONE = 0, ACT_GELU = 1, ACT_SILU = 2, ACT_GELU_TANH = 3 };

enum EpiMode : int {
    EPI_STORE = 0,
    EPI_RESID = 1,
    EPI_STORE_T = 2,
};

struct Epilogue {
    int mode = EPI_STORE;
    int act = ACT_NONE;
    int out_dtype = F32;
    const float* bias = nullptr;
    void* out = nullptr;
    int ldo = 0;
    const float* gamma = nullptr;
    float* resid = nullptr;
    const int* len = nullptr;
    int L = 1;
    const int* row_b = nullptr;
    const float* rowvec = nullptr;
    int rv_ld = 0;
    int ksplit = 1;
    int nt = 0;
    int tr_epilogue = 0;
    int tr_force = -1;
    unsigned long long* ts = nullptr;
};

enum GemmKernel : int { GK_TILED = 0, GK_RING_VEC = 1, GK_RING = 2, GK_REG = 3 };
enum GemmEpiForm : int { GE_LANE = 0, GE_SLAB = 1, GE_TR = 2 };
constexpr int GEMM_CFG_F32_64 = 19, GEMM_CFG_F32_128 = 20;
struct GemmForm {
    int dtype = F32, mode = EPI_STORE;
    int kernel = GK_REG;
    int cfg = 0;
    int bm = 128, bn = 128, wm = 2, wn = 2, nstage = 2, ks = 64, esz = 2;
    int epi = GE_LANE;
    int tr_epilogue = 0;
    int split = 1;
    std::string str() const;
};
GemmForm gemm_form(int dtype, int M, int N, int K, int lda, int ldw, const Epilogue& e, const void* A, const void* W, bool allow_split = true);
void launch_gemm_form(hipStream_t s, const GemmForm& f, const void* A, int lda, const void* W, int ldw, int M, int N, int K,
                      const Epilogue& e, float* workspace);
void launch_gemm(hipStream_t s, int dtype, const void* A, int lda, const void* W, int ldw, int M, int N, int K,
                 const Epilogue& e);
int gemm_splitk_factor(int dtype, int M, int N, int K, const Epilogue& e);
void launch_gemm_splitk(hipStream_t s, int dtype, const void* A, int lda, const void* W, int ldw, int M, int N, int K, const Epilogue& e,
                        int S, float* workspace);

struct FfnArgs {
    const void* xn = nullptr; int ldx = 0;
    const void* wseq = nullptr;
    const float* b1 = nullptr;
    const float* b2 = nullptr;
    const float* gamma = nullptr;
    float* x = nullptr; int ldo = 0;
    int M = 0, I = 0;
    const int* row_b = nullptr;
    const float* rowvec = nullptr; int rv_ld = 0;
    const int* len = nullptr; int L = 1;
    unsigned long long* ts = nullptr;
    int split = 1;
    void* part = nullptr;
    int64_t part_stride = 0;
};
bool ffn_fused_supported(int dtype, int C, int I);
int ffn_split_factor(int dtype, int C, int I);
constexpr int FFN_SPLITS[] = {4, 8, 12};
bool ffn_split_valid(int dtype, int C, int I, int S);
int ffn_split_choose(int dtype, int C, int I, int64_t M);
inline int64_t ffn_split_rows(int64_t M) { return (M + 127) / 128 * 128; }
enum FfnKind : int { FFN_GEMMS = 0, FFN_K4 = 1, FFN_K4_SPLIT = 2 };
enum FfnStage : int { FFN_VOCODER = 1, FFN_ESTIMATOR = 2, FFN_TEXT = 4 };
struct FfnForm {
    int kind = FFN_GEMMS, split = 1;
    bool nt = false;
// ... 73 lines not shown
void launch_repack_frag(hipStream_t s, const void* W, int N, int K, void* Wf);
bool xattn_hs_supported(int dtype, int C, int H, int L, int Lk, int ldk);
void launch_xattn_hs(hipStream_t s, int dtype, const void* xn, int64_t M, const void* WqF, const float* bq, const void* kp, const void* vp, int ldk,
                     const void* WoA, void* part, int64_t part_stride, int B, int L, int Lk, const int* qlen, const int* klen,
                     const int* q_off, const int* k_off, int rope_mode, float rope_base, float rope_gamma, unsigned long long* ts = nullptr,
                     const int* pairs = nullptr );
struct XattnHsForm {
    bool f16 = false;
    int U = 1, kc = 32;
    size_t lds = 0;
    std::string str() const;
};
XattnHsForm xattn_hs_form(int dtype, int C, int H, int B, int L, int Lk, int ldk);
void launch_xattn_hs_pairs(hipStream_t s, const int* qlen, int B, int* pairs);
void launch_rope_rows(hipStream_t s, int dtype, void* x, int ld, int B, int L, const int* len, int groups, int group_stride,
                      int H, int dh, int rope_mode, float rope_base, float rope_gamma, const int* row_off = nullptr );

void launch_embed(hipStream_t s, const int64_t* ids, const float* emb, int vocab, int B, int L, int C, const int* len,
                  float* x, const int* row_off = nullptr );
void launch_mask_to_len(hipStream_t s, const float* mask, int B, int L, int* len);
void launch_ncl_to_rows(hipStream_t s, int out_dtype, const float* in, int B, int C, int L, void* out, int ld_out = 0,
                        const int* len = nullptr, const int* row_off = nullptr );
void launch_euler_ncl(hipStream_t s, const float* prev, const float* v, const float* dt, const int* len, int B, int D, int L, float* out,
                      const int* row_off = nullptr , void* z_rows = nullptr, int z_dtype = 0, int ldz = 0);
void launch_cast(hipStream_t s, int out_dtype, const float* in, int64_t n, void* out);
void launch_add_rowvec(hipStream_t s, float* x, const float* v, int ldv, int B, int L, int C, const int* len);
void launch_time_embed(hipStream_t s, const float* cur, const float* tot, int B, int dim, float scale, float* te);
void launch_scale_len(hipStream_t s, const int* len, int B, int factor, int* out);
void launch_vocoder_in(hipStream_t s, const float* latent, int B, int L, int ld, int ccf, const float* w ,
                       const float* bias, int C, int k, float* x, const int* seqlen = nullptr);
void launch_vocoder_im2col(hipStream_t s, int out_dtype, const float* latent, int B, int L, int ld, int ccf, int k, int kp, void* cols,
                           const int* seqlen = nullptr ,
                           const int* row_off = nullptr );
void launch_unpack_rows(hipStream_t s, const float* src, const int* len, const int* row_off, int B, int T, int W, float* dst);
void launch_trim_len(hipStream_t s, const int* len, int B, int ccf, int T, int rf, int* n_out, int* valid_out, bool tail_form = false);
void launch_unpack_rows_quiet(hipStream_t s, const float* src, const int* valid, const int* row_off, int B, int T, int W, int rf,
                              const float* quiet, const float* edge, float* dst);
void launch_masked_mean(hipStream_t s, int in_dtype, const void* x, int B, int L, int C, const int* len, float* pooled,
                        const int* row_off = nullptr );
void launch_softplus(hipStream_t s, float* x, int n);
void launch_scale(hipStream_t s, float* x, int n, float mul);
void launch_randn_masked(hipStream_t s, uint64_t seed, const int64_t* utt_ids, int B, int D, int L, const int* len,
                         float* xt, const unsigned long long* seed_dev = nullptr );
void launch_mask_ncl(hipStream_t s, float* x, int B, int D, int L, const int* len);
void launch_reciprocal(hipStream_t s, const float* in, int n, float* out);
void launch_bf16_to_f32(hipStream_t s, const uint16_t* in, int64_t n, float* out);
void launch_half_to_f32(hipStream_t s, int in_dtype, const void* in, int64_t n, float* out);
void launch_fill(hipStream_t s, float* x, int n, float v);
void launch_step_counters(hipStream_t s, float* tot , float* cur , float* dt , int B, int steps);
enum OutEnc : int { ENC_F32 = 0, ENC_PCM16 = 1, ENC_PCM24 = 2, ENC_MULAW = 3, ENC_ALAW = 4 };
constexpr int enc_bytes(int enc) {
    return enc == ENC_F32 ? 4 : enc == ENC_PCM16 ? 2 : enc == ENC_PCM24 ? 3 : (enc == ENC_MULAW || enc == ENC_ALAW) ? 1 : 0;
}
template <typename Fn>
inline void with_enc(int enc, const char* who, Fn&& fn) {
    switch (enc) {
        case ENC_F32: fn(std::integral_constant<int, ENC_F32>{}); break;
        case ENC_PCM16: fn(std::integral_constant<int, ENC_PCM16>{}); break;
        case ENC_PCM24: fn(std::integral_constant<int, ENC_PCM24>{}); break;
        case ENC_MULAW: fn(std::integral_constant<int, ENC_MULAW>{}); break;
        case ENC_ALAW: fn(std::integral_constant<int, ENC_ALAW>{}); break;
        default: throw std::invalid_argument(std::string(who) + ": unknown encoding " + std::to_string(enc));
    }
}
struct Dither {
    int mode = DITHER_OFF; uint64_t seed = 0; unsigned kind = DITHER_ROW; const int64_t* ids = nullptr;
// ... 144 lines not shown
```

supertonic_amd/csrc/kernels_gemm.hip:

```cpp
#include "kernels.hpp"
#include "dev_env.hpp"
#include "kernels_dev.hpp"

#include <hip/hip_bf16.h>
#include <stdio.h>
#include <stdlib.h>

namespace stn {

static constexpr int BM = 128, BN = 128, NT = 256;
static constexpr int STAGE_BYTES = (BM + BN) * 128;

__device__ __forceinline__ int xcd_remap(int bid, int nwg) {
    const int q = nwg >> 3, r = nwg & 7, xcd = bid & 7, loc = bid >> 3;
    const int base = xcd < r ? xcd * (q + 1) : r * (q + 1) + (xcd - r) * q;
    return base + loc;
}

template <int MODE, bool F16 = false>
__device__ __forceinline__ void run_epilogue(const Epilogue& e, f32x16 (&acc)[2][2], int m_base, int n_base, int M,
                                             int N, int lane) {
    const int half = lane >> 5, cl = lane & 31;
    float bias[2], gam[2];
    int ncol[2];
// ... 588 lines not shown
                        o.w = (unsigned)(unsigned short)hi[2] | ((unsigned)(unsigned short)hi[3] << 16);
                        *reinterpret_cast<uint4*>(reinterpret_cast<uint16_t*>(e.out) + (size_t)m * e.ldo + nst) = o;
                    }
                }
                __builtin_amdgcn_fence(__ATOMIC_RELEASE, "wavefront");
            }
        }
        if (e.ts && tid == 0) {
            __builtin_amdgcn_s_waitcnt(0);
            unsigned long long* tp = e.ts + (size_t)blockIdx.x * 4;
            tp[0] = t_in; tp[1] = t_first; tp[2] = t_loop; tp[3] = __builtin_readcyclecounter();
        }
        return;
    }

    float* S = reinterpret_cast<float*>(smem);
    constexpr int CG = BN_ / 8;
    constexpr int ROWS_PER_IT = NTHR / CG;
    constexpr int ITER = (WM * 32) / ROWS_PER_IT;
    static_assert(NTHR % CG == 0 && (WM * 32) % ROWS_PER_IT == 0, "epilogue thread map");
    const int half = lane >> 5, cl = lane & 31;
    const int c8 = tid % CG, rbase = tid / CG;
    const int n = n0 + c8 * 8;
    const bool ncol_ok = n < N;
    float bias[8], gam[8];
    {
        float4 b0 = make_float4(0.f, 0.f, 0.f, 0.f), b1 = b0, g0 = make_float4(1.f, 1.f, 1.f, 1.f), g1 = g0;
        if (ncol_ok && e.bias) { b0 = *reinterpret_cast<const float4*>(e.bias + n); b1 = *reinterpret_cast<const float4*>(e.bias + n + 4); }
        if (MODE == EPI_RESID && ncol_ok && e.gamma) { g0 = *reinterpret_cast<const float4*>(e.gamma + n); g1 = *reinterpret_cast<const float4*>(e.gamma + n + 4); }
        bias[0] = b0.x; bias[1] = b0.y; bias[2] = b0.z; bias[3] = b0.w; bias[4] = b1.x; bias[5] = b1.y; bias[6] = b1.z; bias[7] = b1.w;
        gam[0] = g0.x; gam[1] = g0.y; gam[2] = g0.z; gam[3] = g0.w; gam[4] = g1.x; gam[5] = g1.y; gam[6] = g1.z; gam[7] = g1.w;
    }
    const bool to_bf16 = e.out_dtype == BF16;
#pragma unroll
    for (int mi = 0; mi < TM; ++mi) {
        float4 r0[ITER], r1[ITER];
        bool ok[ITER];
        float keep[ITER];
        size_t off[ITER];
        int bq[ITER];
#pragma unroll
        for (int it = 0; it < ITER; ++it) {
            const int srow = rbase + it * ROWS_PER_IT;
            const int m = m0 + ((srow >> 5) * TM + mi) * 32 + (srow & 31);
            ok[it] = ncol_ok && m < M;
            keep[it] = 1.f;
            off[it] = (size_t)m * e.ldo + n;
            bq[it] = 0;
            if (ok[it] && e.row_b) {
                bq[it] = e.row_b[m];
            } else if (ok[it] && (e.len || (MODE == EPI_RESID && e.rowvec))) {
                const int b = m / e.L;
                bq[it] = b;
                if (e.len && m - b * e.L >= e.len[b]) keep[it] = 0.f;
            }
            if (MODE == EPI_RESID) {
                r0[it] = make_float4(0.f, 0.f, 0.f, 0.f); r1[it] = r0[it];
                if (ok[it]) { r0[it] = *reinterpret_cast<const float4*>(e.resid + off[it]); r1[it] = *reinterpret_cast<const float4*>(e.resid + off[it] + 4); }
            }
        }
        __syncthreads();
#pragma unroll
        for (int ni = 0; ni < TN; ++ni)
#pragma unroll
            for (int i = 0; i < 16; ++i) {
                const int srow = wm * 32 + (i & 3) + 8 * (i >> 2) + 4 * half;
                S[srow * BN_ + (wn * TN + ni) * 32 + cl] = acc[mi][ni][i];
            }
        __syncthreads();
#pragma unroll
        for (int it = 0; it < ITER; ++it) {
            const int srow = rbase + it * ROWS_PER_IT;
            const float4 v0 = *reinterpret_cast<const float4*>(S + srow * BN_ + c8 * 8);
            const float4 v1 = *reinterpret_cast<const float4*>(S + srow * BN_ + c8 * 8 + 4);
            if (!ok[it]) continue;
            float v[8] = {v0.x, v0.y, v0.z, v0.w, v1.x, v1.y, v1.z, v1.w};
            if (MODE == EPI_STORE) {
                act8(v, bias, e.act, to_bf16, keep[it]);
                if (e.out_dtype != F32) {
                    uint4 pk;
                    pk.x = (unsigned)cvt16<F16>(v[0]) | ((unsigned)cvt16<F16>(v[1]) << 16);
                    pk.y = (unsigned)cvt16<F16>(v[2]) | ((unsigned)cvt16<F16>(v[3]) << 16);
                    pk.z = (unsigned)cvt16<F16>(v[4]) | ((unsigned)cvt16<F16>(v[5]) << 16);
                    pk.w = (unsigned)cvt16<F16>(v[6]) | ((unsigned)cvt16<F16>(v[7]) << 16);
                    uint4* po = reinterpret_cast<uint4*>(reinterpret_cast<uint16_t*>(e.out) + off[it]);
                    if (e.nt & 1) { const u32x4 pv = {pk.x, pk.y, pk.z, pk.w}; __builtin_nontemporal_store(pv, reinterpret_cast<u32x4*>(po)); }
                    else *po = pk;
// ... 186 lines not shown
            f = gemm_form(dtype, M, N, K, lda, ldw, ep, A, W, false);
            f.mode = e.mode;
            f.split = S;
            return f;
        }
    }
    const bool ring = is_half(dtype) && K % RK == 0;
    const void* optr = e.mode == EPI_RESID ? static_cast<const void*>(e.resid) : e.out;
    const bool vec_ok = e.mode <= EPI_RESID && N % 8 == 0 && e.ldo % 8 == 0 && !misaligned16(optr) && !misaligned16(e.bias) &&
                        !misaligned16(e.gamma);
    const int cfg = vec_ok && (ring || dtype == F32) ? tiled_cfg(dtype, M, N, K) : 0;
    if (cfg > 0) {
        const TileShape& t = kTiles[cfg];
        f.kernel = GK_TILED;
        f.cfg = cfg;
        f.bm = t.bm; f.bn = t.bn; f.wm = t.wm; f.wn = t.wn; f.nstage = t.ns; f.ks = t.ks; f.esz = t.esz;
        if (dtype == F32) {
            f.tr_epilogue = e.tr_epilogue;
        } else if (e.tr_force >= 0) {
            f.tr_epilogue = e.tr_force != 0;
        } else {
            static int g_tr = -2;
            if (g_tr == -2) { const char* c = stn::dev_env("STN_GEMM_TR"); g_tr = c ? atoi(c) : 1; }
            f.tr_epilogue = g_tr == 2 || (g_tr == 1 && (cfg == 11 || cfg == 8 || cfg == 12 || cfg == 13 || cfg == 14 || cfg == 18));
        }
        f.epi = (e.mode == EPI_STORE && f.esz == 2 && e.out_dtype != F32 && e.len == nullptr && f.tr_epilogue) ? GE_TR : GE_SLAB;
        return f;
    }
    f.kernel = ring && vec_ok ? GK_RING_VEC : ring ? GK_RING : GK_REG;
    f.epi = f.kernel == GK_RING_VEC ? GE_SLAB : GE_LANE;
    return f;
}

std::string GemmForm::str() const {
    char b[128];
    const char* ep = epi == GE_TR ? "tr" : epi == GE_SLAB ? "slab" : "lane";
    char sp[16] = "";
    if (split > 1) snprintf(sp, sizeof sp, "splitk%d+", split);
    if (kernel == GK_TILED) {
        char c[8] = "";
        if (cfg <= 18) snprintf(c, sizeof c, " cfg%d", cfg);
        snprintf(b, sizeof b, "%stiled<%d,%d,%d,%d,%d,%d,%d>%s %s", sp, bm, bn, wm, wn, nstage, ks, esz, c, ep);
    } else {
        snprintf(b, sizeof b, "%s%s %s", sp, kernel == GK_RING_VEC ? "ring_vec" : kernel == GK_RING ? "ring" : "reg", ep);
    }
    return b;
}

template <int MODE>
static void launch_untiled(hipStream_t s, const GemmForm& f, const void* A, int lda, const void* W, int ldw, int M, int N, int K,
                           const Epilogue& e) {
    const int tiles_m = (M + BM - 1) / BM, tiles_n = (N + BN - 1) / BN, ntiles = tiles_m * tiles_n;
    const uint16_t* A16 = static_cast<const uint16_t*>(A);
    const uint16_t* W16 = static_cast<const uint16_t*>(W);
#define STN_LAUNCH_H(F16_)                                                                                                       \
    if (f.kernel == GK_RING_VEC) {                                                                                               \
        if constexpr (MODE <= EPI_RESID)                                                                                         \
            STN_KLAUNCH((gemm_bf16_ring_kernel<MODE, true, F16_>), dim3(ntiles), dim3(NT), 0, s, A16, lda, W16, ldw, M, N, K,      \
                        tiles_n, ntiles, e);                                                                                      \
    } else if (f.kernel == GK_RING)                                                                                              \
        STN_KLAUNCH((gemm_bf16_ring_kernel<MODE, false, F16_>), dim3(ntiles), dim3(NT), 0, s, A16, lda, W16, ldw, M, N, K,         \
                    tiles_n, ntiles, e);                                                                                          \
    else                                                                                                                         \
        STN_KLAUNCH((gemm_bf16_kernel<MODE, F16_>), dim3(ntiles), dim3(NT), 0, s, A16, lda, W16, ldw, M, N, K, tiles_n, ntiles, e);
    if (f.dtype == F16) { STN_LAUNCH_H(true) }
    else if (f.dtype == BF16) { STN_LAUNCH_H(false) }
    else
        STN_KLAUNCH(gemm_f32_kernel<MODE>, dim3(ntiles), dim3(NT), 0, s, static_cast<const float*>(A), lda, static_cast<const float*>(W),
                    ldw, M, N, K, tiles_n, ntiles, e);
#undef STN_LAUNCH_H
}

void launch_gemm_form(hipStream_t s, const GemmForm& f, const void* A, int lda, const void* W, int ldw, int M, int N, int K,
                      const Epilogue& e, float* workspace) {
    if (M <= 0 || N <= 0) return;
    if (f.mode != e.mode) throw std::invalid_argument("launch_gemm_form: the form was made for another epilogue mode");
    if (f.split > 1) {
        if (!workspace || misaligned16(workspace)) throw std::invalid_argument("launch_gemm_form: a split-K form needs a 16-byte aligned workspace of split * M * N floats");
        Epilogue ep;
        ep.mode = EPI_STORE; ep.out_dtype = F32; ep.out = workspace; ep.ldo = N; ep.ksplit = f.split;
        GemmForm fp = f;
        fp.mode = EPI_STORE;
        fp.split = 1;
        launch_gemm_form(s, fp, A, lda, W, ldw, M, N, K, ep, nullptr);
        const int64_t n4 = (int64_t)M * (N / 4);
        const dim3 grid((unsigned)((n4 + 255) / 256));
        if (e.mode == EPI_RESID) STN_KLAUNCH(splitk_reduce_kernel<EPI_RESID>, grid, dim3(256), 0, s, workspace, f.split, M, N, e);
        else STN_KLAUNCH(splitk_reduce_kernel<EPI_STORE>, grid, dim3(256), 0, s, workspace, f.split, M, N, e);
        return;
    }
    if (f.kernel == GK_TILED) {
        Epilogue et = e;
        et.tr_epilogue = f.tr_epilogue;
        if (e.mode == EPI_STORE) launch_tiled_cfg<EPI_STORE>(s, f.dtype, f.cfg, A, lda, W, ldw, M, N, K, et);
        else if (e.mode == EPI_RESID) launch_tiled_cfg<EPI_RESID>(s, f.dtype, f.cfg, A, lda, W, ldw, M, N, K, et);
        else throw std::invalid_argument("launch_gemm_form: the tiled kernels have no transposing epilogue");
        return;
    }
    switch (e.mode) {
        case EPI_STORE: launch_untiled<EPI_STORE>(s, f, A, lda, W, ldw, M, N, K, e); break;
        case EPI_RESID: launch_untiled<EPI_RESID>(s, f, A, lda, W, ldw, M, N, K, e); break;
        default: launch_untiled<EPI_STORE_T>(s, f, A, lda, W, ldw, M, N, K, e); break;
    }
}

void launch_gemm(hipStream_t s, int dtype, const void* A, int lda, const void* W, int ldw, int M, int N, int K,
                 const Epilogue& e) {
    if (M <= 0 || N <= 0) return;
    launch_gemm_form(s, gemm_form(dtype, M, N, K, lda, ldw, e, A, W, false), A, lda, W, ldw, M, N, K, e, nullptr);
// ... 12 lines not shown
```

supertonic_amd/csrc/kernels_layout.hip:

```cpp
#include "kernels.hpp"
#include "kernels_dev.hpp"

#include <type_traits>

namespace stn {

__global__ void embed_kernel(const int64_t* __restrict__ ids, const float* __restrict__ emb, int vocab, int L, int C,
                             const int* __restrict__ len, float* __restrict__ x, const int* __restrict__ row_off) {
    const int row = blockIdx.x, b = row / L, t = row - b * L;
    if (row_off && t >= len[b]) return;
    const int64_t id = ids[row];
    const bool ok = t < len[b] && id >= 0 && id < vocab;
    const int C4 = C >> 2;
    float4* o = reinterpret_cast<float4*>(x) + (row_off ? (int64_t)row_off[b] + t : (int64_t)row) * C4;
    const float4* e = reinterpret_cast<const float4*>(emb) + (ok ? id : 0) * C4;
    for (int c = threadIdx.x; c < C4; c += blockDim.x) {
        float4 v = make_float4(0.f, 0.f, 0.f, 0.f);
        if (ok) v = e[c];
        o[c] = v;
    }
}
void launch_embed(hipStream_t s, const int64_t* ids, const float* emb, int vocab, int B, int L, int C, const int* len,
                  float* x, const int* row_off) {
    if (B * L == 0) return;
// ... 439 lines not shown
                                                                float* __restrict__ dst) {
    const int lane = threadIdx.x & 63;
    const int wave = __builtin_amdgcn_readfirstlane((int)(threadIdx.x >> 6));
    const int64_t r0 = ((int64_t)blockIdx.x * 4 + wave) * UNPACK_RW;
    if (r0 >= nrows) return;
    const float4* sp[UNPACK_RW];
#pragma unroll
    for (int i = 0; i < UNPACK_RW; ++i) {
        const int64_t r = r0 + i < nrows ? r0 + i : nrows - 1;
        const int b = (int)(r / T), t = (int)(r - (int64_t)b * T);
        if (t < valid[b]) sp[i] = reinterpret_cast<const float4*>(src) + ((int64_t)row_off[b] + t) * W4;
        else if (t >= T - rf) sp[i] = reinterpret_cast<const float4*>(edge) + (int64_t)(t - (T - rf)) * W4;
        else sp[i] = reinterpret_cast<const float4*>(quiet);
    }
    float4* d4 = reinterpret_cast<float4*>(dst) + r0 * W4;
    for (int c = lane; c < W4; c += 64) {
        float4 v[UNPACK_RW];
#pragma unroll
        for (int i = 0; i < UNPACK_RW; ++i) v[i] = sp[i][c];
#pragma unroll
        for (int i = 0; i < UNPACK_RW; ++i)
            if (r0 + i < nrows) d4[(int64_t)i * W4 + c] = v[i];
    }
}
void launch_unpack_rows_quiet(hipStream_t s, const float* src, const int* valid, const int* row_off, int B, int T, int W, int rf,
                              const float* quiet, const float* edge, float* dst) {
    const int64_t nrows = (int64_t)B * T;
    if (nrows == 0 || W == 0) return;
    if (W % 4) { throw std::invalid_argument("unpack_rows needs W % 4 == 0"); }
    STN_KLAUNCH(unpack_rows_quiet_kernel, dim3((unsigned)((nrows + 4 * UNPACK_RW - 1) / (4 * UNPACK_RW))), dim3(256), 0, s, src, valid, row_off, T,
                W / 4, rf, quiet, edge, nrows, dst);
}

__global__ void mask_ncl_kernel(float* __restrict__ x, int D, int L, int64_t n, const int* __restrict__ len) {
    const int64_t i = (int64_t)blockIdx.x * blockDim.x + threadIdx.x;
    if (i >= n) return;
    const int t = (int)(i % L);
    const int b = (int)(i / ((int64_t)D * L));
    if (t >= len[b]) x[i] = 0.f;
}
void launch_mask_ncl(hipStream_t s, float* x, int B, int D, int L, const int* len) {
    const int64_t n = (int64_t)B * D * L;
    if (n == 0) return;
    STN_KLAUNCH(mask_ncl_kernel, dim3((unsigned)((n + 255) / 256)), dim3(256), 0, s, x, D, L, n, len);
}

}
```

Before: 47500.

## Scatter vocoder head GEMM rows directly into waveform and pack length tables

The vocoder head GEMM's tiled slab epilogue gains a packed-row destination map, so each output row is written straight to its (batch, time) slot in the waveform buffer instead of going to a temporary and being unpacked afterwards. A new fill_rows kernel writes only the padding and quiet-tail rows beyond each sequence's valid length. Per-batch length tables (offsets, valid counts) are built on the host into one pinned table, replacing separate row_map and trim kernels and separate pinned buffers. Profiling spans are also added around several layout kernels. The epilogue adds a per-row batch search and bounds check, and falls back to the old path when the GEMM form is not a tiled fp32 slab store.

Result: faster. 48110, median of 6 (+1.3%).

```diff
diff --git a/include/stn.h b/include/stn.h
--- a/include/stn.h
+++ b/include/stn.h
@@ -289,12 +289,16 @@
 int stn_op_dwconv_ln_ragged(stn_handle* h, int dtype, int B, int L, int C, int k, int dil, const float* x,
                             const float* w , const float* bias, const float* ln_g, const float* ln_b,
                             const int32_t* seqlen , float* y);
+int stn_op_gemm_rows(stn_handle* h, int dtype, int M, int N, int K, const float* A, const float* W, const float* bias_or_null, int B,
+                     const int32_t* rows, const int32_t* valid, int T, float* out, int64_t out_elems, char* form, size_t form_cap);
 int stn_op_dwconv_ln_ex(stn_handle* h, int dtype, int B, int L, int C, int k, int dil, const float* x, int64_t x_rows,
                         const float* w_or_null , const float* bias_or_null, const float* ln_g, const float* ln_b,
                         const int32_t* seqlen_or_null, int packed, int ln_only, float* y, int64_t y_rows, char* form, size_t form_cap);
 int stn_op_dwconv_ln_tail(stn_handle* h, int dtype, int B, int L, int C, int k, int dil, const float* x, int64_t x_rows,
                           const float* w , const float* bias, const float* ln_g, const float* ln_b, const int32_t* seqlen,
                           const float* tail , int T, int rf, float* y, int64_t y_rows, char* form, size_t form_cap);
+int64_t stn_dbg_len_tables(int B, const int32_t* llen, int ve_rows, int with_pairs, int vo_form, int ccf, int T, int rf, int32_t* layout,
+                           int32_t* out, int64_t out_n);
 int stn_dbg_dwconv_ln_form(int dtype, int B, int L, int C, int k, int packed, char* out, size_t cap);
 int stn_op_fold_ln(stn_handle* h, int dtype, int M, int C, int S, const float* part, const float* b2, const float* gamma,
                    const float* rowvec_or_null, const int32_t* row_b_or_null, int nseq, const float* ln_g, const float* ln_b, float* x,
diff --git a/supertonic_amd/binding.py b/supertonic_amd/binding.py
--- a/supertonic_amd/binding.py
+++ b/supertonic_amd/binding.py
@@ -16,6 +16,7 @@
 EPI_STORE, EPI_RESID, EPI_STORE_T = 0, 1, 2
 FFN_VOCODER, FFN_ESTIMATOR, FFN_TEXT = 1, 2, 4
 LAYOUT_ROW_MAP, LAYOUT_NCL_TO_ROWS, LAYOUT_EULER_NCL, LAYOUT_UNPACK_ROWS, LAYOUT_EMBED, LAYOUT_MASKED_MEAN, LAYOUT_IM2COL, LAYOUT_VOCODER_IN = range(8)
+LAYOUT_FILL_ROWS, LAYOUT_HS_PAIRS, LAYOUT_TRIM_LEN = 8, 9, 10
 ENC_F32, ENC_PCM16, ENC_PCM24, ENC_MULAW, ENC_ALAW = 0, 1, 2, 3, 4
 ENCODINGS = {"f32": ENC_F32, "pcm16": ENC_PCM16, "pcm24": ENC_PCM24, "mulaw": ENC_MULAW, "alaw": ENC_ALAW}
 ENCODING_NAMES = {v: k for k, v in ENCODINGS.items()}
@@ -571,6 +572,7 @@
     L.stn_op_dwconv_ln.argtypes = [vp, ci, ci, ci, ci, ci, ci, _f32p, _f32p, _f32p, _f32p, _f32p, _f32p]
     L.stn_op_dwconv_ln_ragged.argtypes = [vp, ci, ci, ci, ci, ci, ci, _f32p, _f32p, _f32p, _f32p, _f32p, _i32p, _f32p]
     L.stn_op_attention.argtypes = [vp, ci, ci, ci, ci, ci, ci, _f32p, _f32p, _f32p, vp, vp, ci, _f32p]
+    L.stn_op_gemm_rows.argtypes = [vp, ci, ci, ci, ci, _f32p, _f32p, vp, ci, _i32p, _i32p, ci, _f32p, ctypes.c_int64, ctypes.c_char_p, ctypes.c_size_t]
     L.stn_op_dwconv_ln_ex.argtypes = [vp, ci, ci, ci, ci, ci, ci, _f32p, ctypes.c_int64, vp, vp, _f32p, _f32p, vp, ci, ci, _f32p, ctypes.c_int64,
                                       ctypes.c_char_p, ctypes.c_size_t]
     L.stn_op_dwconv_ln_tail.argtypes = [vp, ci, ci, ci, ci, ci, ci, _f32p, ctypes.c_int64, _f32p, _f32p, _f32p, _f32p, _i32p, _f32p, ci, ci, _f32p,
@@ -579,6 +581,8 @@
     L.stn_dbg_resample_form.restype = ctypes.c_int
     L.stn_dbg_dwconv_ln_form.argtypes = [ci, ci, ci, ci, ci, ci, ctypes.c_char_p, ctypes.c_size_t]
     L.stn_dbg_dwconv_ln_form.restype = ctypes.c_int
+    L.stn_dbg_len_tables.argtypes = [ci, _i32p, ci, ci, ci, ci, ci, ci, _i32p, ctypes.c_void_p, ctypes.c_int64]
+    L.stn_dbg_len_tables.restype = ctypes.c_int64
     L.stn_op_fold_ln.argtypes = [vp, ci, ci, ci, ci, _f32p, _f32p, _f32p, vp, vp, ci, _f32p, _f32p, _f32p, _f32p]
     L.stn_op_layout.argtypes = [vp, ci, ci, _i32p, ci, vp, ctypes.c_int64, vp, ctypes.c_int64, vp, ctypes.c_int64, vp, ctypes.c_int64, vp, ci,
                                 vp, ctypes.c_int64, vp, ctypes.c_int64, vp, ctypes.c_int64]
@@ -1172,6 +1176,30 @@
     return buf.value.decode()
 
 
+LEN_VO_NONE, LEN_VO_2RF, LEN_VO_TAIL, LEN_VO_SCALED = range(4)
+
+
+def len_tables(llen, ve_rows=0, with_pairs=False, vo_form=LEN_VO_NONE, ccf=6, T=0, rf=0):
+    llen = _c(llen, np.int32)
+    B = len(llen)
+    lay = np.zeros(9, np.int32)
+    args = (B, llen, int(ve_rows), int(bool(with_pairs)), int(vo_form), int(ccf), int(T), int(rf))
+    tot = load().stn_dbg_len_tables(*args, lay, None, 0)
+    if tot < 0:
+        raise StnError(int(tot), "stn_dbg_len_tables: bad argument")
+    out = np.full(tot, -12345, np.int32)
+    out[:2] = 7
+    assert load().stn_dbg_len_tables(*args, lay, out.ctypes.data, out.size) == tot
+    assert out[0] == 7 and out[1] == 7
+    names = ("seed", "llen", "ve_off", "ve_row_b", "pairs", "vo_n", "vo_valid", "vo_off")
+    sizes = {"llen": B, "ve_off": B + 1, "ve_row_b": int(ve_rows), "pairs": B + 2, "vo_n": B, "vo_valid": B, "vo_off": B + 1}
+    res = {"total": int(tot)}
+    for i, n in enumerate(names):
+        if n != "seed" and lay[i] >= 0:
+            res[n] = out[lay[i]:lay[i] + sizes[n]].copy()
+    return res
+
+
 def fold_dwconv_ln_form(dtype, B, L, C, k, dil, S, rowvec=True, run_frames=0):
     buf = ctypes.create_string_buffer(96)
     r = load().stn_dbg_fold_dwconv_ln_form(_DTYPES[dtype], int(B), int(L), int(C), int(k), int(dil), int(S), int(bool(rowvec)), int(run_frames),
@@ -2141,6 +2169,19 @@
                                             _c(g, np.float32), _c(b, np.float32), y))
         return y
 
+    def op_gemm_rows(self, A, W, out, rows, valid, T, bias=None, dtype=None):
+        A = _c(A, np.float32)
+        W = _c(W, np.float32)
+        rows = _c(rows, np.int32)
+        valid = _c(valid, np.int32)
+        o_r = np.array(out, dtype=np.float32, order="C", copy=True)
+        _b, bp = _opt(bias, np.float32)
+        form = ctypes.create_string_buffer(96)
+        self._ck(self._lib.stn_op_gemm_rows(self._h, self.dtype if dtype is None else _DTYPES[dtype], A.shape[0], W.shape[0], A.shape[1],
+                                            A.reshape(-1), W.reshape(-1), bp, len(rows), rows, valid, int(T), o_r.reshape(-1), o_r.size, form,
+                                            ctypes.sizeof(form)))
+        return o_r, form.value.decode()
+
     def op_dwconv_ln_ex(self, x, w, bias, g, b, dil, out, B, L, seqlen=None, packed=False, ln_only=False, dtype=None):
         x = _c(x, np.float32)
         o_r = np.array(out, dtype=np.float32, order="C", copy=True)
diff --git a/supertonic_amd/csrc/api.cpp b/supertonic_amd/csrc/api.cpp
--- a/supertonic_amd/csrc/api.cpp
+++ b/supertonic_amd/csrc/api.cpp
@@ -935,6 +935,24 @@
                  for (int i = 0; i < B; ++i) need(seqlen[i] >= 0 && seqlen[i] <= L, "stn_op_dwconv_ln_ragged: seqlen out of [0, L]");
                  h->eng->op_dwconv_ln(dtype, B, L, C, k, dil, x, w, bias, g, b, y, seqlen); })
 }
+static void gemm_rows_checked(stn_handle* h, int dtype, int M, int N, int K, const float* A, const float* W, const float* bias, int B,
+                              const int32_t* rows, const int32_t* valid, int T, float* out, int64_t out_elems, char* form, size_t form_cap) {
+    need(M > 0 && N > 0 && K > 0 && A && W && out && rows && valid && B > 0 && B <= 1024 && T > 0, "stn_op_gemm_rows: bad argument");
+    need(dtype == STN_DTYPE_F32 || dtype == STN_DTYPE_BF16 || dtype == STN_DTYPE_F16, "stn_op_gemm_rows: unknown dtype");
+    need(K % (dtype != STN_DTYPE_F32 ? 8 : 4) == 0, "stn_op_gemm_rows: K must be a multiple of 8 (16-bit) / 4 (f32)");
+    int64_t tot = 0;
+    for (int b = 0; b < B; ++b) {
+        need(rows[b] >= 0 && rows[b] <= T && valid[b] >= 0 && valid[b] <= rows[b], "stn_op_gemm_rows: needs 0 <= valid[b] <= rows[b] <= T");
+        tot += rows[b];
+    }
+    need(tot <= M && out_elems >= (int64_t)B * T * N, "stn_op_gemm_rows: needs sum rows <= M and out_elems >= B*T*N");
+    const std::string f = h->eng->op_gemm_rows(dtype, M, N, K, A, W, bias, B, rows, valid, T, out, out_elems);
+    if (form && form_cap) std::snprintf(form, form_cap, "%s", f.c_str());
+}
+int stn_op_gemm_rows(stn_handle* h, int dtype, int M, int N, int K, const float* A, const float* W, const float* bias, int B, const int32_t* rows,
+                     const int32_t* valid, int T, float* out, int64_t out_elems, char* form, size_t form_cap) {
+    STN_TRY(h, gemm_rows_checked(h, dtype, M, N, K, A, W, bias, B, rows, valid, T, out, out_elems, form, form_cap))
+}
 static void dwconv_ln_ex_checked(stn_handle* h, int dtype, int B, int L, int C, int k, int dil, const float* x, int64_t x_rows, const float* w,
                                  const float* bias, const float* g, const float* b, const int32_t* seqlen, int packed, int ln_only, float* y,
                                  int64_t y_rows, char* form, size_t form_cap) {
@@ -978,6 +996,27 @@
                           int64_t y_rows, char* form, size_t form_cap) {
     STN_TRY(h, dwconv_ln_tail_checked(h, dtype, B, L, C, k, dil, x, x_rows, w, bias, g, b, seqlen, tail, T, rf, y, y_rows, form, form_cap))
 }
+int64_t stn_dbg_len_tables(int B, const int32_t* llen, int ve_rows, int with_pairs, int vo_form, int ccf, int T, int rf, int32_t* layout,
+                           int32_t* out, int64_t out_n) {
+    if (B < 1 || B > 1024 || !llen || ve_rows < 0 || vo_form < stn::LEN_VO_NONE || vo_form > stn::LEN_VO_SCALED || ccf < 1 || T < 0 || rf < 0) return STN_ERR_INVALID;
+    int64_t tot = 0;
+    for (int b = 0; b < B; ++b) {
+        if (llen[b] < 0 || llen[b] > (1 << 20)) return STN_ERR_INVALID;
+        tot += llen[b];
+    }
+    if (ve_rows > 0 && tot > ve_rows) return STN_ERR_INVALID;
+    if (with_pairs && ve_rows == 0) return STN_ERR_INVALID;
+    const stn::LenTables t = stn::len_tables_layout(B, ve_rows, with_pairs != 0, vo_form);
+    if (layout) {
+        const int v[9] = {t.seed, t.llen, t.ve_off, t.ve_row_b, t.pairs, t.vo_n, t.vo_valid, t.vo_off, t.total};
+        std::memcpy(layout, v, sizeof v);
+    }
+    if (out) {
+        if (out_n < t.total) return STN_ERR_INVALID;
+        stn::len_tables_build(t, llen, B, ve_rows, with_pairs != 0, vo_form, ccf, T, rf, out);
+    }
+    return t.total;
+}
 int stn_dbg_dwconv_ln_form(int dtype, int B, int L, int C, int k, int packed, char* out, size_t cap) {
     if (B < 1 || L < 1 || C < 1 || k < 1 || !(k & 1) || (dtype != STN_DTYPE_F32 && dtype != STN_DTYPE_BF16 && dtype != STN_DTYPE_F16)) return STN_ERR_INVALID;
     std::string f;
@@ -997,8 +1036,8 @@
 int stn_op_layout(stn_handle* h, int which, int dtype, const int32_t* p, int n_p, const float* a, int64_t a_n, const float* b, int64_t b_n,
                   const float* c, int64_t c_n, const int64_t* ids, int64_t ids_n, const int32_t* len, int packed, float* out, int64_t out_n,
                   float* out2, int64_t out2_n, int32_t* iout, int64_t iout_n) {
-    static const int n_params[8] = {3, 4, 5, 3, 4, 3, 6, 6};
-    STN_TRY(h, { need(which >= 0 && which < 8 && p && n_p == n_params[which], "stn_op_layout: unknown kernel or parameter count");
+    static const int n_params[11] = {3, 4, 5, 3, 4, 3, 6, 6, 5, 1, 5};
+    STN_TRY(h, { need(which >= 0 && which < 11 && p && n_p == n_params[which], "stn_op_layout: unknown kernel or parameter count");
                  need(dtype == STN_DTYPE_F32 || dtype == STN_DTYPE_BF16 || dtype == STN_DTYPE_F16, "stn_op_layout: unknown dtype");
                  need(a_n >= 0 && b_n >= 0 && c_n >= 0 && ids_n >= 0 && out_n >= 0 && out2_n >= 0 && iout_n >= 0 && (a || !a_n) && (b || !b_n) && (c || !c_n) &&
                           (ids || !ids_n) && (out || !out_n) && (out2 || !out2_n) && (iout || !iout_n),
diff --git a/supertonic_amd/csrc/engine.cpp b/supertonic_amd/csrc/engine.cpp
--- a/supertonic_amd/csrc/engine.cpp
+++ b/supertonic_amd/csrc/engine.cpp
@@ -161,9 +161,7 @@
     for (auto& sp : spans_) { (void)hipEventDestroy(sp.a); (void)hipEventDestroy(sp.b); }
     for (auto ev : ev_pool_) (void)hipEventDestroy(ev);
     drop_graphs();
-    if (pin_llen_) (void)hipHostFree(pin_llen_);
-    if (pin_seed_) (void)hipHostFree(pin_seed_);
-    if (seed_dev_) (void)hipFree(seed_dev_);
+    if (pin_tab_) (void)hipHostFree(pin_tab_);
     rs_release();
     fl_release();
     xp_release();
@@ -778,7 +776,11 @@
     const Arena::Mark mk = ar_.mark();
     const int Dp = (D + 63) / 64 * 64;
     void* z = z_rows ? z_rows : act_alloc(M * Dp);
-    if (!(z_rows && z_ready)) launch_ncl_to_rows(s_, dt_, noisy, B, D, L, z, Dp, llen, roff);
+    if (!(z_rows && z_ready)) {
+        if (prof_on_) prof_begin("ncl_to_rows", 0.0, (double)B * D * L * 4.0 + (double)M * Dp * esz);
+        launch_ncl_to_rows(s_, dt_, noisy, B, D, L, z, Dp, llen, roff);
+        if (prof_on_) prof_end();
+    }
     const FfnForm ff = ffn_plan(FFN_ESTIMATOR, C, a.ve_hidden, M, 0, rg != nullptr, a.ve_kernel, 1 << std::max(0, a.ve_dilated - 1));
     const bool split = ff.kind == FFN_K4_SPLIT;
     FoldState fs;
@@ -863,7 +865,9 @@
     float* vel = f32_alloc(M * D);
     Epilogue eo; eo.mode = EPI_STORE; eo.out_dtype = F32; eo.out = vel; eo.ldo = D;
     gemm("gemm_out", dt_, xn, C, linear("ve.out"), (int)M, eo);
+    if (prof_on_) prof_begin("euler", 2.0 * M * D, (double)M * D * 4.0 + (double)B * D * L * 8.0 + ((z_rows && z_next) ? (double)M * Dp * esz : 0.0));
     launch_euler_ncl(s_, noisy, vel, dtv, llen, B, D, L, denoised, roff, (z_rows && z_next) ? z_rows : nullptr, dt_, Dp);
+    if (prof_on_) prof_end();
     ar_.release(mk);
 }
 
@@ -1047,7 +1051,7 @@
     return rows;
 }
 
-void Engine::vocoder_dev(int B, int L, const float* latent, float* wav, const int* vlen, int vrows, const int* valid, bool tails) {
+void Engine::vocoder_dev(int B, int L, const float* latent, float* wav, const int* vlen, int vrows, const int* valid, bool tails, const int* voff) {
     stage_ = "vo";
     const stn_arch& a = a_;
     const int C = a.vo_dim, T = L * a.chunk_compress_factor;
@@ -1057,9 +1061,13 @@
     const int64_t M = packed ? (int64_t)vrows : (int64_t)B * T;
     const Arena::Mark mk = ar_.mark();
     Ragged rg;
-    if (packed) {
+    if (packed && voff) {
+        rg.off = voff; rg.rows = vrows;
+    } else if (packed) {
         int* off = static_cast<int*>(ar_.alloc(sizeof(int) * (size_t)(B + 1)));
+        if (prof_on_) prof_begin("row_map", 0.0, (double)(2 * B + 1) * 4.0);
         launch_row_map(s_, vlen, B, off, nullptr);
+        if (prof_on_) prof_end();
         rg.off = off; rg.rows = vrows;
     }
     const Ragged* rgp = packed ? &rg : nullptr;
@@ -1067,8 +1075,10 @@
     if (is_half(dt_)) {
         const int kp = (a.latent_dim * a.vo_in_kernel + 63) / 64 * 64;
         void* cols = act_alloc(M * kp);
+        if (prof_on_) prof_begin("im2col", 0.0, (double)B * L * a.latent_dim * a.chunk_compress_factor * 4.0 + (double)M * kp * 2.0);
         launch_vocoder_im2col(s_, dt_, latent, B, L, a.latent_dim, a.chunk_compress_factor, a.vo_in_kernel, kp, cols, vlen,
                               packed ? rg.off : nullptr);
+        if (prof_on_) prof_end();
         Linear lin;
         lin.w = tensor("vo.in_gemm.w"); lin.b = vecf("vo.in.b"); lin.N = C; lin.K = kp;
         Epilogue ei; ei.mode = EPI_STORE; ei.out_dtype = F32; ei.out = x; ei.ldo = C;
@@ -1098,15 +1108,29 @@
     }
     void* xn = act_alloc(M * C);
     const LNorm ln = lnorm("vo.out_ln");
+    if (prof_on_) prof_begin("layernorm", (double)M * C * 8, (double)M * C * (4.0 + (is_half(dt_) ? 2.0 : 4.0)));
     launch_layernorm(s_, dt_, x, M, C, ln.g, ln.b, a.ln_eps, xn);
+    if (prof_on_) prof_end();
     if (packed) {
-        float* wp = f32_alloc(M * a.base_chunk_size);
-        Epilogue e; e.mode = EPI_STORE; e.out_dtype = F32; e.out = wp; e.ldo = a.base_chunk_size;
-        gemm("gemm_head", dt_, xn, C, linear("vo.head"), (int)M, e);
-        if (prof_on_) prof_begin("unpack_rows", 0.0, ((double)M + (double)B * T) * a.base_chunk_size * 4.0);
-        if (valid) launch_unpack_rows_quiet(s_, wp, valid, rg.off, B, T, a.base_chunk_size, vo_rf_, vc.quiet, vc.edge, wav);
-        else launch_unpack_rows(s_, wp, vlen, rg.off, B, T, a.base_chunk_size, wav);
-        if (prof_on_) prof_end();
+        const int W = a.base_chunk_size;
+        const Linear& head = linear("vo.head");
+        Epilogue e; e.mode = EPI_STORE; e.out_dtype = F32; e.out = wav; e.ldo = W; e.bias = head.b;
+        e.map_off = rg.off; e.map_valid = valid ? valid : vlen; e.map_B = B; e.map_T = T;
+        if (gemm_form_maps_rows(gemm_form(dt_, (int)M, head.N, head.K, C, head.K, e, xn, head.w.as(dt_)))) {
+            if (prof_on_) prof_begin("fill_rows", 0.0, std::max(0.0, (double)B * T - (double)M) * W * 4.0);
+            if (valid) launch_fill_rows(s_, valid, B, T, W, vo_rf_, vc.quiet, vc.edge, wav);
+            else launch_fill_rows(s_, vlen, B, T, W, 0, nullptr, nullptr, wav);
+            if (prof_on_) prof_end();
+            gemm("gemm_head", dt_, xn, C, head, (int)M, e);
+        } else {
+            float* wp = f32_alloc(M * W);
+            Epilogue ep; ep.mode = EPI_STORE; ep.out_dtype = F32; ep.out = wp; ep.ldo = W;
+            gemm("gemm_head", dt_, xn, C, head, (int)M, ep);
+            if (prof_on_) prof_begin("unpack_rows", 0.0, ((double)M + (double)B * T) * W * 4.0);
+            if (valid) launch_unpack_rows_quiet(s_, wp, valid, rg.off, B, T, W, vo_rf_, vc.quiet, vc.edge, wav);
+            else launch_unpack_rows(s_, wp, vlen, rg.off, B, T, W, wav);
+            if (prof_on_) prof_end();
+        }
     } else {
         Epilogue e; e.mode = EPI_STORE; e.out_dtype = F32; e.out = wav; e.ldo = a.base_chunk_size; e.len = vlen; e.L = T;
         gemm("gemm_head", dt_, xn, C, linear("vo.head"), (int)M, e);
diff --git a/supertonic_amd/csrc/engine.hpp b/supertonic_amd/csrc/engine.hpp
--- a/supertonic_amd/csrc/engine.hpp
+++ b/supertonic_amd/csrc/engine.hpp
@@ -11,6 +11,7 @@
 #include <vector>
 
 #include "../../include/stn_arch.h"
+#include "host/len_tables.hpp"
 #include "host/join_plan.hpp"
 #include "host/pause_plan.hpp"
 #include "host/pitch.hpp"
@@ -153,7 +154,7 @@
                      bool z_ready = false ,
                      bool z_next = false );
     void vocoder_dev(int B, int L, const float* latent, float* wav, const int* vlen = nullptr, int vrows = 0,
-                     const int* valid = nullptr, bool tails = false);
+                     const int* valid = nullptr, bool tails = false, const int* voff = nullptr);
     int vocoder_receptive_field() const;
     void prepare_xattn_weights();
     std::unordered_map<const void*, const void*> frag_w_;
@@ -186,7 +187,9 @@
         float* style_ttl = nullptr; size_t ttl_cap = 0;
         float* style_dp = nullptr; size_t dp_cap = 0;
         float* dur = nullptr; size_t dur_cap = 0;
-        int* llen = nullptr; size_t llen_cap = 0;
+        int* llen = nullptr;
+        int* tab = nullptr; size_t tab_cap = 0;
+        LenTables tl;
         int64_t* utt_ids = nullptr; size_t utt_cap = 0;
         float* noise = nullptr; size_t noise_cap = 0;
         float* xt[2] = {nullptr, nullptr}; size_t xt_cap[2] = {0, 0};
@@ -399,6 +402,8 @@
                             int rope_mode, int pairs_mode, int64_t part_stride, float* part, int64_t part_elems, int* pairs_out);
     void op_attention(int dtype, int B, int Lq, int Lk, int H, int dh, const float* q, const float* k, const float* v,
                       const int* qlen, const int* klen, int rope_mode, float* o);
+    std::string op_gemm_rows(int dtype, int M, int N, int K, const float* A, const float* W, const float* bias, int B, const int* rows,
+                             const int* valid, int T, float* out, int64_t out_elems);
     void op_dwconv_ln(int dtype, int B, int L, int C, int k, int dil, const float* x, const float* w, const float* bias,
                       const float* g, const float* b, float* y, const int* seqlen = nullptr );
     std::string op_dwconv_ln_ex(int dtype, int B, int L, int C, int k, int dil, const float* x, int64_t x_rows, const float* w, const float* bias,
@@ -559,9 +564,10 @@
     int tail_rows(int B, int L) const;
     int vocoder_rows(int B, int L, int* form) const;
     long graph_replays_ = 0;
-    int* pin_llen_ = nullptr; size_t pin_llen_cap_ = 0;
-    unsigned long long* pin_seed_ = nullptr;
+    int* pin_tab_ = nullptr; size_t pin_tab_cap_ = 0;
+    size_t pin_tab_n_ = 0;
     bool pin_valid_ = false;
+    std::vector<int32_t> h_tab_;
     unsigned long long* seed_dev_ = nullptr;
     int final_xt_ = 0;
     struct FetchSlot { unsigned char* dev = nullptr; unsigned char* pin = nullptr; size_t cap = 0, n = 0; int enc = ENC_PCM16; hipEvent_t ready = nullptr, done = nullptr; bool busy = false; std::vector<float> dur; };
diff --git a/supertonic_amd/csrc/engine_batch.cpp b/supertonic_amd/csrc/engine_batch.cpp
--- a/supertonic_amd/csrc/engine_batch.cpp
+++ b/supertonic_amd/csrc/engine_batch.cpp
@@ -46,7 +46,6 @@
     ensure(b.style_ttl, b.ttl_cap, n_ttl);
     ensure(b.style_dp, b.dp_cap, n_dp);
     ensure(b.dur, b.dur_cap, (size_t)B);
-    ensure(b.llen, b.llen_cap, (size_t)B);
     ensure(b.utt_ids, b.utt_cap, (size_t)B);
     if (Lt != Lt_in) {
         STN_HIP(hipMemsetAsync(b.ids, 0, sizeof(int64_t) * B * Lt, s_));
@@ -163,34 +162,42 @@
     ensure(b.xt[0], b.xt_cap[0], nx);
     ensure(b.xt[1], b.xt_cap[1], nx);
     ensure(b.wav, b.wav_cap, nw);
-    if ((size_t)B > pin_llen_cap_) {
-        if (pin_llen_) { sync(); drop_graphs(); (void)hipHostFree(pin_llen_); pin_llen_ = nullptr; }
-        const size_t cap = std::max<size_t>((size_t)B, 1024);
-        STN_HIP(hipHostMalloc(reinterpret_cast<void**>(&pin_llen_), sizeof(int) * cap, hipHostMallocDefault));
-        pin_llen_cap_ = cap;
+    int ve_rows = 0;
+    if (packed_rows_ok(B)) for (int v : b.h_llen) ve_rows += v;
+    if (shape_buckets_) ve_rows = (int)bucket_up(ve_rows, 64);
+    int vform = VO_DENSE;
+    const int tr_rows = vocoder_rows(B, L, &vform);
+    const int tab_vo = vo_ragged_ ? LEN_VO_SCALED : !tr_rows ? LEN_VO_NONE : vform == VO_TRIM_TAIL ? LEN_VO_TAIL : LEN_VO_2RF;
+    const bool tab_pairs = ve_rows > 0 && fused_xattn_ && is_half(dt_) && B >= 2;
+    b.tl = len_tables_layout(B, ve_rows, tab_pairs, tab_vo);
+    h_tab_.assign((size_t)b.tl.total, 0);
+    len_tables_build(b.tl, b.h_llen.data(), B, ve_rows, tab_pairs, tab_vo, a.chunk_compress_factor, L * a.chunk_compress_factor, vo_rf_, h_tab_.data());
+    const unsigned long long seed64 = (unsigned long long)noise_seed;
+    std::memcpy(h_tab_.data() + b.tl.seed, &seed64, sizeof seed64);
+    ensure(b.tab, b.tab_cap, (size_t)b.tl.total);
+    b.llen = b.tab + b.tl.llen;
+    seed_dev_ = reinterpret_cast<unsigned long long*>(b.tab + b.tl.seed);
+    if ((size_t)b.tl.total > pin_tab_cap_) {
+        if (pin_tab_) { sync(); drop_graphs(); (void)hipHostFree(pin_tab_); pin_tab_ = nullptr; }
+        const size_t cap = std::max<size_t>((size_t)b.tl.total + (size_t)b.tl.total / 4, (size_t)1024 * (64 + 8));
+        STN_HIP(hipHostMalloc(reinterpret_cast<void**>(&pin_tab_), sizeof(int) * cap, hipHostMallocDefault));
+        pin_tab_cap_ = cap;
         pin_valid_ = false;
     }
-    if (!pin_seed_) {
-        STN_HIP(hipHostMalloc(reinterpret_cast<void**>(&pin_seed_), sizeof(unsigned long long), hipHostMallocDefault));
-        STN_HIP(hipMalloc(reinterpret_cast<void**>(&seed_dev_), sizeof(unsigned long long)));
-        pin_valid_ = false;
-    }
-    if (!pin_valid_ || !std::equal(b.h_llen.begin(), b.h_llen.end(), pin_llen_) || *pin_seed_ != (unsigned long long)noise_seed) {
+    if (!pin_valid_ || pin_tab_n_ != h_tab_.size() || !std::equal(h_tab_.begin(), h_tab_.end(), pin_tab_)) {
         sync();
-        std::copy(b.h_llen.begin(), b.h_llen.end(), pin_llen_);
-        *pin_seed_ = (unsigned long long)noise_seed;
+        std::copy(h_tab_.begin(), h_tab_.end(), pin_tab_);
+        pin_tab_n_ = h_tab_.size();
         pin_valid_ = true;
     }
 
     ensure_time_cond(total_step, B);
     GraphKey key;
     key.B = B; key.Lt = Lt; key.L = L; key.steps = total_step; key.noise = b.have_noise; key.ragged = vo_ragged_; key.xattn = fused_xattn_;
-    key.ffn = fused_ffn_; key.gen = b.gen; key.wgen = wgen_; key.pin = pin_llen_;
-    key.rows = 0;
-    if (packed_rows_ok(B)) for (int v : b.h_llen) key.rows += v;
-    if (shape_buckets_) key.rows = (int)bucket_up(key.rows, 64);
+    key.ffn = fused_ffn_; key.gen = b.gen; key.wgen = wgen_; key.pin = pin_tab_;
+    key.rows = ve_rows;
     last_ve_rows_ = key.rows ? key.rows : (int64_t)B * L;
-    key.vrows = vocoder_rows(B, L, &key.vform);
+    key.vrows = tr_rows; key.vform = vform;
     if (shape_buckets_) key.vrows = (int)bucket_up(key.vrows, 64 * a.chunk_compress_factor);
     key.trows = tpk ? b.trows : 0;
     last_vo_rows_ = (int64_t)B * L * a.chunk_compress_factor;
@@ -297,8 +304,7 @@
     const stn_arch& a = a_;
     const int B = b.B, Lt = b.Lt, L = b.L, D = a.latent_dim * a.chunk_compress_factor;
     const size_t nx = (size_t)B * D * L;
-    STN_HIP(hipMemcpyAsync(b.llen, pin_llen_, sizeof(int) * B, hipMemcpyHostToDevice, s_));
-    STN_HIP(hipMemcpyAsync(seed_dev_, pin_seed_, sizeof(unsigned long long), hipMemcpyHostToDevice, s_));
+    STN_HIP(hipMemcpyAsync(b.tab, pin_tab_, sizeof(int) * (size_t)b.tl.total, hipMemcpyHostToDevice, s_));
     Ragged trg;
     const bool tpk = packed_text_ok(B) && b.trows > 0;
     if (tpk) { trg.off = b.toff; trg.rows = b.trows; }
@@ -308,7 +314,10 @@
         STN_HIP(hipMemcpyAsync(b.xt[0], b.noise, nx * 4, hipMemcpyDeviceToDevice, s_));
         launch_mask_ncl(s_, b.xt[0], B, D, L, b.llen);
     } else {
+        stage_ = "ve";
+        if (prof_on_) prof_begin("noise", 0.0, (double)nx * 4.0);
         launch_randn_masked(s_, 0, b.utt_ids, B, D, L, b.llen, b.xt[0], seed_dev_);
+        if (prof_on_) prof_end();
     }
     VeCtx c = ve_prepare_dev(B, Lt, text_rows, b.style_ttl, b.tlen, trgp, true);
     text_gate_ = [this, &c, &b, &take_text_rows, B, Lt, text_rows, trgp]() {
@@ -329,14 +338,14 @@
         rg.rows = 0;
         for (int v : b.h_llen) rg.rows += v;
         if (shape_buckets_) rg.rows = (int)bucket_up(rg.rows, 64);
-        int* off = static_cast<int*>(ar_.alloc(sizeof(int) * (size_t)(B + 1)));
-        int* row_b = static_cast<int*>(ar_.alloc(sizeof(int) * (size_t)std::max(rg.rows, 1)));
-        launch_row_map(s_, b.llen, B, off, row_b, rg.rows);
+        if (b.tl.ve_off < 0 || b.tl.ve_row_b + rg.rows > b.tl.total) throw std::logic_error("batch_run: no row map in the length tables");
+        const int* off = b.tab + b.tl.ve_off;
+        const int* row_b = b.tab + b.tl.ve_row_b;
         rg.off = off; rg.row_b = row_b;
         rg.fold_run = fold_run_frames(b.h_llen.data(), B, n_cu_);
         if (fused_xattn_ && is_half(dt_) && B >= 2) {
-            int* pairs = static_cast<int*>(ar_.alloc(sizeof(int) * (size_t)(B + 2)));
-            launch_xattn_hs_pairs(s_, b.llen, B, pairs);
+            if (b.tl.pairs < 0) throw std::logic_error("batch_run: no pairing in the length tables");
+            const int* pairs = b.tab + b.tl.pairs;
             rg.hs_pairs = pairs;
         }
         rgp = &rg;
@@ -352,11 +361,7 @@
     }
     final_xt_ = cur;
     const int* vlen = nullptr;
-    if (vo_ragged_) {
-        int* v = static_cast<int*>(ar_.alloc(sizeof(int) * B));
-        launch_scale_len(s_, b.llen, B, a.chunk_compress_factor, v);
-        vlen = v;
-    }
+    if (vo_ragged_) vlen = b.tab + b.tl.vo_n;
     int vrows = 0;
     const int* valid = nullptr;
     bool tails = false;
@@ -365,12 +370,10 @@
         if (shape_buckets_) vrows = (int)bucket_up(vrows, 64 * a.chunk_compress_factor);
     } else if (int vform = VO_DENSE; int tr = vocoder_rows(B, L, &vform)) {
         if (shape_buckets_) tr = (int)bucket_up(tr, 64 * a.chunk_compress_factor);
-        int* n_dev = static_cast<int*>(ar_.alloc(sizeof(int) * B));
-        int* v_dev = static_cast<int*>(ar_.alloc(sizeof(int) * B));
-        launch_trim_len(s_, b.llen, B, a.chunk_compress_factor, L * a.chunk_compress_factor, vo_rf_, n_dev, v_dev, vform == VO_TRIM_TAIL);
-        vlen = n_dev; valid = v_dev; vrows = tr; tails = vform == VO_TRIM_TAIL;
-    }
-    vocoder_dev(B, L, b.xt[cur], b.wav, vlen, vrows, valid, tails);
+        vlen = b.tab + b.tl.vo_n; valid = b.tab + b.tl.vo_valid; vrows = tr; tails = vform == VO_TRIM_TAIL;
+    }
+    if (vlen && b.tl.vo_n < 0) throw std::logic_error("batch_run: no vocoder extents in the length tables");
+    vocoder_dev(B, L, b.xt[cur], b.wav, vlen, vrows, valid, tails, vlen ? b.tab + b.tl.vo_off : nullptr);
     STN_HIP(hipGetLastError());
 }
 
diff --git a/supertonic_amd/csrc/engine_ops.cpp b/supertonic_amd/csrc/engine_ops.cpp
--- a/supertonic_amd/csrc/engine_ops.cpp
+++ b/supertonic_amd/csrc/engine_ops.cpp
@@ -70,6 +70,37 @@
     const GemmForm f = gemm_form(dtype, M, N, K, K, K, e, pa, pw);
     launch_gemm_form(s_, f, pa, K, pw, K, M, N, K, e, f.split > 1 ? f32_alloc((int64_t)f.split * M * N) : nullptr);
     if (o16) launch_half_to_f32(s_, out_dtype, o16, out_elems, dO);
+    STN_HIP(hipMemcpyAsync(out, dO, (size_t)out_elems * 4, hipMemcpyDeviceToHost, s_));
+    sync();
+    return f.str();
+}
+
+std::string Engine::op_gemm_rows(int dtype, int M, int N, int K, const float* A, const float* W, const float* bias, int B, const int* rows,
+                                 const int* valid, int T, float* out, int64_t out_elems) {
+    STN_HIP(hipSetDevice(device_));
+    ar_.reset();
+    float* dA = up(ar_, s_, A, (size_t)M * K);
+    float* dW = up(ar_, s_, W, (size_t)N * K);
+    const void* pa = dA;
+    const void* pw = dW;
+    if (is_half(dtype)) {
+        void* a16 = ar_.alloc((size_t)M * K * 2);
+        void* w16 = ar_.alloc((size_t)N * K * 2);
+        launch_cast(s_, dtype, dA, (int64_t)M * K, a16);
+        launch_cast(s_, dtype, dW, (int64_t)N * K, w16);
+        pa = a16; pw = w16;
+    }
+    float* dO = up(ar_, s_, out, (size_t)out_elems);
+    const int* drows = up(ar_, s_, rows, (size_t)B);
+    int* off = static_cast<int*>(ar_.alloc(sizeof(int) * (size_t)(B + 1)));
+    launch_row_map(s_, drows, B, off, nullptr);
+    Epilogue e;
+    e.mode = EPI_STORE; e.out_dtype = F32; e.out = dO; e.ldo = N;
+    e.bias = bias ? up(ar_, s_, bias, (size_t)N) : nullptr;
+    e.map_off = off; e.map_valid = up(ar_, s_, valid, (size_t)B); e.map_B = B; e.map_T = T;
+    const GemmForm f = gemm_form(dtype, M, N, K, K, K, e, pa, pw, false);
+    launch_gemm_form(s_, f, pa, K, pw, K, M, N, K, e, nullptr);
+    STN_HIP(hipGetLastError());
     STN_HIP(hipMemcpyAsync(out, dO, (size_t)out_elems * 4, hipMemcpyDeviceToHost, s_));
     sync();
     return f.str();
@@ -746,6 +777,41 @@
         STN_HIP(hipMemcpyAsync(out, d, (size_t)out_n * 4, hipMemcpyDeviceToHost, s_));
         break;
     }
+    case 8: {
+        const int B = p[0], T = p[1], W = p[2], rf = p[3], zeros = p[4];
+        need(T > 0 && W > 0 && W % 4 == 0 && rf >= 0 && rf <= T && out, "fill_rows: bad shape");
+        check_len(B, T, true);
+        need(out_n >= (int64_t)B * T * W, "fill_rows: buffer too small");
+        need(zeros || (a && a_n >= W && (rf == 0 || (b && b_n >= (int64_t)rf * W))), "fill_rows: the quiet rule needs quiet [W] and edge [rf][W]");
+        const int* dlen = up(ar_, s_, len, (size_t)B);
+        const float* dq = zeros ? nullptr : up(ar_, s_, a, (size_t)a_n);
+        const float* de = (zeros || rf == 0) ? nullptr : up(ar_, s_, b, (size_t)b_n);
+        float* d = up(ar_, s_, out, (size_t)out_n);
+        launch_fill_rows(s_, dlen, B, T, W, rf, dq, de, d);
+        STN_HIP(hipMemcpyAsync(out, d, (size_t)out_n * 4, hipMemcpyDeviceToHost, s_));
+        break;
+    }
+    case 9: {
+        const int B = p[0];
+        check_len(B, 1 << 20, true);
+        need(iout && iout_n >= 2 * ((B + 1) / 2), "hs_pairs: iout too small");
+        const int* dlen = up(ar_, s_, len, (size_t)B);
+        int* d = up(ar_, s_, iout, (size_t)iout_n);
+        launch_xattn_hs_pairs(s_, dlen, B, d);
+        STN_HIP(hipMemcpyAsync(iout, d, (size_t)iout_n * 4, hipMemcpyDeviceToHost, s_));
+        break;
+    }
+    case 10: {
+        const int B = p[0], ccf = p[1], T = p[2], rf = p[3], tail_form = p[4];
+        need(ccf > 0 && T > 0 && rf >= 0, "trim_len: bad shape");
+        check_len(B, T / ccf, true);
+        need(iout && iout_n >= 2 * (int64_t)B, "trim_len: iout too small");
+        const int* dlen = up(ar_, s_, len, (size_t)B);
+        int* d = up(ar_, s_, iout, (size_t)iout_n);
+        launch_trim_len(s_, dlen, B, ccf, T, rf, d, d + B, tail_form != 0);
+        STN_HIP(hipMemcpyAsync(iout, d, (size_t)iout_n * 4, hipMemcpyDeviceToHost, s_));
+        break;
+    }
     default: need(false, "unknown kernel");
     }
     STN_HIP(hipGetLastError());
diff --git a/supertonic_amd/csrc/host/len_tables.cpp b/supertonic_amd/csrc/host/len_tables.cpp
--- /dev/null
+++ b/supertonic_amd/csrc/host/len_tables.cpp
@@ -0,0 +1,70 @@
+#include "len_tables.hpp"
+
+#include <algorithm>
+#include <numeric>
+#include <vector>
+
+namespace stn {
+
+LenTables len_tables_layout(int B, int ve_rows, bool with_pairs, int vo_form) {
+    LenTables t;
+    int at = t.llen + B;
+    if (ve_rows > 0) {
+        t.ve_off = at; at += B + 1;
+        t.ve_row_b = at; at += ve_rows;
+    }
+    if (with_pairs) { t.pairs = at; at += B + 2; }
+    if (vo_form != LEN_VO_NONE) {
+        t.vo_n = at; at += B;
+        t.vo_valid = at; at += B;
+        t.vo_off = at; at += B + 1;
+    }
+    t.total = (at + 3) & ~3;
+    return t;
+}
+
+void len_tables_build(const LenTables& t, const int* llen, int B, int ve_rows, bool with_pairs, int vo_form, int ccf, int T, int rf, int32_t* out) {
+    std::fill(out + t.llen, out + t.total, 0);
+    std::copy(llen, llen + B, out + t.llen);
+    if (t.ve_off >= 0) {
+        int32_t* off = out + t.ve_off;
+        int32_t* row_b = out + t.ve_row_b;
+        off[0] = 0;
+        for (int b = 0; b < B; ++b) {
+            off[b + 1] = off[b] + llen[b];
+            std::fill(row_b + off[b], row_b + std::min(off[b + 1], ve_rows), b);
+        }
+    }
+    if (with_pairs && t.pairs >= 0) {
+        std::vector<int> sorted(B);
+        std::iota(sorted.begin(), sorted.end(), 0);
+        std::stable_sort(sorted.begin(), sorted.end(), [&](int x, int y) { return llen[x] < llen[y]; });
+        int32_t* pairs = out + t.pairs;
+        const int G = (B + 1) / 2;
+        for (int i = 0; i < G; ++i) {
+            pairs[2 * i] = sorted[B - 1 - i];
+            pairs[2 * i + 1] = B - 1 - i > i ? sorted[i] : -1;
+        }
+    }
+    if (t.vo_n >= 0) {
+        int32_t* n = out + t.vo_n;
+        int32_t* valid = out + t.vo_valid;
+        int32_t* off = out + t.vo_off;
+        off[0] = 0;
+        for (int b = 0; b < B; ++b) {
+            const int l6 = llen[b] * ccf;
+            if (vo_form == LEN_VO_SCALED) {
+                n[b] = valid[b] = l6;
+            } else if (vo_form == LEN_VO_TAIL) {
+                n[b] = valid[b] = l6 + rf < T ? l6 + rf : T;
+            } else {
+                const bool trim = l6 + 2 * rf <= T;
+                n[b] = trim ? l6 + 2 * rf : T;
+                valid[b] = trim ? l6 + rf : T;
+            }
+            off[b + 1] = off[b] + n[b];
+        }
+    }
+}
+
+}
diff --git a/supertonic_amd/csrc/host/len_tables.hpp b/supertonic_amd/csrc/host/len_tables.hpp
--- /dev/null
+++ b/supertonic_amd/csrc/host/len_tables.hpp
@@ -0,0 +1,28 @@
+#pragma once
+#include <cstdint>
+
+namespace stn {
+
+enum LenVoForm : int {
+    LEN_VO_NONE = 0,
+    LEN_VO_2RF = 1,
+    LEN_VO_TAIL = 2,
+    LEN_VO_SCALED = 3,
+};
+
+struct LenTables {
+    int seed = 0;
+    int llen = 2;
+    int ve_off = -1;
+    int ve_row_b = -1;
+    int pairs = -1;
+    int vo_n = -1;
+    int vo_valid = -1;
+    int vo_off = -1;
+    int total = 0;
+};
+
+LenTables len_tables_layout(int B, int ve_rows, bool with_pairs, int vo_form);
+void len_tables_build(const LenTables& t, const int* llen, int B, int ve_rows, bool with_pairs, int vo_form, int ccf, int T, int rf, int32_t* out);
+
+}
diff --git a/supertonic_amd/csrc/kernels.hpp b/supertonic_amd/csrc/kernels.hpp
--- a/supertonic_amd/csrc/kernels.hpp
+++ b/supertonic_amd/csrc/kernels.hpp
@@ -82,6 +82,9 @@
     const int* row_b = nullptr;
     const float* rowvec = nullptr;
     int rv_ld = 0;
+    const int* map_off = nullptr;
+    const int* map_valid = nullptr;
+    int map_B = 0, map_T = 0;
     int ksplit = 1;
     int nt = 0;
     int tr_epilogue = 0;
@@ -105,6 +108,7 @@
 GemmForm gemm_form(int dtype, int M, int N, int K, int lda, int ldw, const Epilogue& e, const void* A, const void* W, bool allow_split = true);
 void launch_gemm_form(hipStream_t s, const GemmForm& f, const void* A, int lda, const void* W, int ldw, int M, int N, int K,
                       const Epilogue& e, float* workspace);
+bool gemm_form_maps_rows(const GemmForm& f);
 void launch_gemm(hipStream_t s, int dtype, const void* A, int lda, const void* W, int ldw, int M, int N, int K,
                  const Epilogue& e);
 int gemm_splitk_factor(int dtype, int M, int N, int K, const Epilogue& e);
@@ -244,6 +248,7 @@
 void launch_vocoder_im2col(hipStream_t s, int out_dtype, const float* latent, int B, int L, int ld, int ccf, int k, int kp, void* cols,
                            const int* seqlen = nullptr ,
                            const int* row_off = nullptr );
+void launch_fill_rows(hipStream_t s, const int* valid, int B, int T, int W, int rf, const float* quiet, const float* edge, float* dst);
 void launch_unpack_rows(hipStream_t s, const float* src, const int* len, const int* row_off, int B, int T, int W, float* dst);
 void launch_trim_len(hipStream_t s, const int* len, int B, int ccf, int T, int rf, int* n_out, int* valid_out, bool tail_form = false);
 void launch_unpack_rows_quiet(hipStream_t s, const float* src, const int* valid, const int* row_off, int B, int T, int W, int rf,
diff --git a/supertonic_amd/csrc/kernels_gemm.hip b/supertonic_amd/csrc/kernels_gemm.hip
--- a/supertonic_amd/csrc/kernels_gemm.hip
+++ b/supertonic_amd/csrc/kernels_gemm.hip
@@ -644,8 +644,27 @@
         gam[0] = g0.x; gam[1] = g0.y; gam[2] = g0.z; gam[3] = g0.w; gam[4] = g1.x; gam[5] = g1.y; gam[6] = g1.z; gam[7] = g1.w;
     }
     const bool to_bf16 = e.out_dtype == BF16;
+    int map_b0 = 0, map_lo0 = 0, map_hi0 = 0, map_vl0 = 0, map_hi1 = 0, map_vl1 = 0;
+    if (MODE == EPI_STORE && e.map_off) {
+        const int Bm = e.map_B, step = (Bm + 63) >> 6;
+        const int i0 = lane * step;
+        const int o0 = i0 < Bm ? e.map_off[i0] : 0;
+        const int c0 = __popcll(__ballot(i0 < Bm && o0 <= m0));
+        int bq0 = (c0 - 1) * step;
+        if (step > 1) {
+            const int i1 = bq0 + lane;
+            const bool in1 = lane < step && i1 < Bm;
+            const int o1 = in1 ? e.map_off[i1] : 0;
+            bq0 += __popcll(__ballot(in1 && o1 <= m0)) - 1;
+        }
+        map_b0 = __builtin_amdgcn_readfirstlane(bq0);
+        const int b1 = map_b0 + 1 < Bm ? map_b0 + 1 : Bm - 1;
+        map_lo0 = e.map_off[map_b0]; map_hi0 = e.map_off[map_b0 + 1]; map_vl0 = e.map_valid[map_b0];
+        map_hi1 = e.map_off[b1 + 1]; map_vl1 = e.map_valid[b1];
+    }
 #pragma unroll
     for (int mi = 0; mi < TM; ++mi) {
+        int mb = map_b0, mlo = map_lo0, mhi = map_hi0, mvl = map_vl0;
         float4 r0[ITER], r1[ITER];
         bool ok[ITER];
         float keep[ITER];
@@ -665,6 +684,13 @@
                 const int b = m / e.L;
                 bq[it] = b;
                 if (e.len && m - b * e.L >= e.len[b]) keep[it] = 0.f;
+            }
+            if (MODE == EPI_STORE && e.map_off && ok[it]) {
+                if (mb == map_b0 && m >= mhi && mb + 1 < e.map_B) { ++mb; mlo = mhi; mhi = map_hi1; mvl = map_vl1; }
+                while (m >= mhi && mb + 1 < e.map_B) { ++mb; mlo = mhi; mhi = e.map_off[mb + 1]; mvl = e.map_valid[mb]; }
+                const int t = m - mlo;
+                ok[it] = t < mvl;
+                off[it] = ((size_t)mb * e.map_T + t) * e.ldo + n;
             }
             if (MODE == EPI_RESID) {
                 r0[it] = make_float4(0.f, 0.f, 0.f, 0.f); r1[it] = r0[it];
@@ -917,6 +943,8 @@
     return f;
 }
 
+bool gemm_form_maps_rows(const GemmForm& f) { return f.kernel == GK_TILED && f.epi == GE_SLAB && f.split == 1 && f.mode == EPI_STORE; }
+
 std::string GemmForm::str() const {
     char b[128];
     const char* ep = epi == GE_TR ? "tr" : epi == GE_SLAB ? "slab" : "lane";
@@ -960,6 +988,8 @@
                       const Epilogue& e, float* workspace) {
     if (M <= 0 || N <= 0) return;
     if (f.mode != e.mode) throw std::invalid_argument("launch_gemm_form: the form was made for another epilogue mode");
+    if (e.map_off && !(gemm_form_maps_rows(f) && e.out_dtype == F32 && !e.len && e.map_valid && e.map_B > 0 && e.map_T > 0))
+        throw std::invalid_argument("launch_gemm_form: a packed-row destination map needs the tiled fp32 slab store, no row mask, and valid / B / T");
     if (f.split > 1) {
         if (!workspace || misaligned16(workspace)) throw std::invalid_argument("launch_gemm_form: a split-K form needs a 16-byte aligned workspace of split * M * N floats");
         Epilogue ep;
diff --git a/supertonic_amd/csrc/kernels_layout.hip b/supertonic_amd/csrc/kernels_layout.hip
--- a/supertonic_amd/csrc/kernels_layout.hip
+++ b/supertonic_amd/csrc/kernels_layout.hip
@@ -495,6 +495,30 @@
                 W / 4, rf, quiet, edge, nrows, dst);
 }
 
+constexpr int FILL_WG = 8;
+__global__ __launch_bounds__(256) void fill_rows_kernel(const int* __restrict__ valid, int T, int W4, int rf, const float* __restrict__ quiet,
+                                                        const float* __restrict__ edge, float* __restrict__ dst) {
+    const int b = blockIdx.x, lane = threadIdx.x & 63;
+    const int w = (int)blockIdx.y * 4 + (int)(threadIdx.x >> 6), nw = (int)gridDim.y * 4;
+    const int v0 = valid[b];
+    float4* d4 = reinterpret_cast<float4*>(dst) + (int64_t)b * T * W4;
+    for (int c = lane; c < W4; c += 64) {
+        const float4 q = quiet ? reinterpret_cast<const float4*>(quiet)[c] : make_float4(0.f, 0.f, 0.f, 0.f);
+        for (int t = v0 + w; t < T; t += nw) {
+            float4 v = q;
+            if (quiet && t >= T - rf) v = reinterpret_cast<const float4*>(edge)[(int64_t)(t - (T - rf)) * W4 + c];
+            d4[(int64_t)t * W4 + c] = v;
+        }
+    }
+}
+void launch_fill_rows(hipStream_t s, const int* valid, int B, int T, int W, int rf, const float* quiet, const float* edge, float* dst) {
+    if (B <= 0 || T <= 0 || W == 0) return;
+    if (W % 4) { throw std::invalid_argument("fill_rows needs W % 4 == 0"); }
+    if (quiet && rf > 0 && !edge) { throw std::invalid_argument("fill_rows: the quiet rule needs the edge tail"); }
+    if (rf < 0 || rf > T) { throw std::invalid_argument("fill_rows: rf outside [0, T]"); }
+    STN_KLAUNCH(fill_rows_kernel, dim3((unsigned)B, FILL_WG), dim3(256), 0, s, valid, T, W / 4, rf, quiet, quiet ? edge : nullptr, dst);
+}
+
 __global__ void mask_ncl_kernel(float* __restrict__ x, int D, int L, int64_t n, const int* __restrict__ len) {
     const int64_t i = (int64_t)blockIdx.x * blockDim.x + threadIdx.x;
     if (i >= n) return;
```
